# TinyMPC/TinyMPC

Measured on AMD Instinct MI355X. Metric: QP solves/sec (+ ADMM iters/sec), 64k-batch quadrotor hover, higher is better.
Workload: dtype f64; 1 GPU; quadrotor_hovering (nx=12, nu=4, N=10), 65536 identical instances per GPU, closed-loop MPC steps from a cold start (BASELINE configs[1]); batch_per_gpu=65536, total_batch=65536, parallelism=batch-sharded x1, mpc_steps_per_launch=8, stats_exchange=none (one rank), launcher=plain process

## Files before the change

tinympc_amd/csrc/admm_kernel.hip.h:

```cpp
#pragma once
#include <hip/hip_runtime.h>
#include <stdint.h>

namespace tinympc_amd {

enum : int {
    VEC_CB = 0,
    VEC_CF = 1,
    VEC_QR = 2,
    VEC_SMASK = 3,
    VEC_NIM = 4,
    VEC_SOCFLAG = 5,
    VEC_CONE_BASE = 6,
    VEC_CONE_MU = 7,
    VEC_RHO = 8,
    VEC_LINFLAG = 9,
    VEC_TLINFLAG = 10,
    VEC_COUNT = 16,
};
struct LaneTab {
    int cols, lw;
    constexpr int MB() const { return 0; }
    constexpr int MF1() const { return cols * lw; }
    constexpr int MF2() const { return 2 * cols * lw; }
    constexpr int PT() const { return 3 * cols * lw; }
    constexpr int VEC() const { return 4 * cols * lw; }
    constexpr int BOUNDS() const { return VEC() + VEC_COUNT * lw; }
    constexpr int het_doubles() const { return BOUNDS(); }
    constexpr int lin_offset(int N) const { return BOUNDS() + 2 * N * lw; }
    constexpr int tlin_offset(int N, int kmax) const { return lin_offset(N) + 3 * kmax * lw; }
    constexpr int doubles(int N, int kmax) const { return tlin_offset(N, kmax) + 3 * N * kmax * lw; }
};
constexpr LaneTab ROW_TAB{16, 16};
enum : int {
    TAB_MB = ROW_TAB.MB(), TAB_MF1 = ROW_TAB.MF1(), TAB_MF2 = ROW_TAB.MF2(), TAB_PT = ROW_TAB.PT(), TAB_VEC = ROW_TAB.VEC(),
    TAB_BOUNDS = ROW_TAB.BOUNDS(),
};
enum : int { LIN_KMAX = 4, LIN_KMAX_BIG = 32 };
enum : int {
    ATAB_AT = 0,
    ATAB_DK = 256,
    ATAB_DP = 512,
    ATAB_DC1 = 768,
    ATAB_DC2 = 1024,
    ATAB_DOUBLES = 1280,
};
static inline int tab_lin_offset(int N) { return ROW_TAB.lin_offset(N); }
static inline int tab_tlin_offset(int N, int kmax = LIN_KMAX) { return ROW_TAB.tlin_offset(N, kmax); }
static inline int tab_doubles(int N, int kmax = LIN_KMAX) { return ROW_TAB.doubles(N, kmax); }

struct SolveArgs {
    const double* tab;
    const double* x0;
    const double* ref;
    double* prim;
    double* slack;
    double* dual;
    double* slack_prev;
    double* cslack;
    double* cdual;
    int4* status;
    double* resid;
    double* x0_next;
    double* dbg_qr;
    double* dbg_pd;
    uint2* accum;
    int* iter_log;
    double* u0_log;
    double rho, tol_pri, tol_dua;
    int batch, max_iter, check_termination;
    int steps;
    const double* traj;
    const int* traj_offsets;
    int traj_points, traj_step0;
    int reset_duals;
    const double* het_tabs;
    double *lslack, *ldual, *tlslack, *tldual;
    int n_lin, n_tlin;
    int cold, store_mask;
    const int* index;
    const int* count;
    int iter_base;
    int* next_index;
    int* next_count;
    double *arho, *aK, *aP, *aC1, *aC2;
    const double* atab;
    double arho_min, arho_max;
    int aclip;
    int ref_shared;
    int* work_counter;
    int reverse;
    const int* perm;
    int perm_count;
    double* vz_stream;
    int pf_mask, pf_shards, pf_static;
    union {
        unsigned* pf_counter;
        const double* inst_bounds;
        const double* inst_lin;
        const double* inst_cones;
    };
    unsigned pf_base[8];
};
static_assert(sizeof(SolveArgs) == 472 && __builtin_offsetof(SolveArgs, het_tabs) == 208 && __builtin_offsetof(SolveArgs, pf_mask) == 416 &&
              __builtin_offsetof(SolveArgs, pf_counter) == 432 && __builtin_offsetof(SolveArgs, pf_base) == 440, "SolveArgs: size and offsets are fixed");

#define DPP_FMA(acc, src, m, lane, bank) "v_fmac_f64_dpp %[" acc "], %[" src "], %[" m "] row_newbcast:" lane " row_mask:0xf bank_mask:" bank "\n\t"
#define DPP_REP1(S) S(0, 0)
#define DPP_REP2(S) DPP_REP1(S) S(1, 1)
#define DPP_REP3(S) DPP_REP2(S) S(2, 0)
#define DPP_REP4(S) DPP_REP3(S) S(3, 1)
#define DPP_REP5(S) DPP_REP4(S) S(4, 0)
#define DPP_REP6(S) DPP_REP5(S) S(5, 1)
#define DPP_REP7(S) DPP_REP6(S) S(6, 0)
#define DPP_REP8(S) DPP_REP7(S) S(7, 1)
#define DPP_REP9(S) DPP_REP8(S) S(8, 0)
#define DPP_REP10(S) DPP_REP9(S) S(9, 1)
#define DPP_REP11(S) DPP_REP10(S) S(10, 0)
#define DPP_REP12(S) DPP_REP11(S) S(11, 1)
#define DPP_REP13(S) DPP_REP12(S) S(12, 0)
#define DPP_REP14(S) DPP_REP13(S) S(13, 1)
#define DPP_REP15(S) DPP_REP14(S) S(14, 0)
#define DPP_REP16(S) DPP_REP15(S) S(15, 1)
#define DPP_REP_(K, S) DPP_REP##K(S)
#define DPP_REP(K, S) DPP_REP_(K, S)
#define DPP_ROW_M(k, p) , [m##k] "v"(m[k])
#define DPP_ROW_A(k, p) , [a##k] "v"(ma[k])
#define DPP_ROW_B(k, p) , [b##k] "v"(mb_[k])
#define RING2_COL(k, p) DPP_FMA("a" #p, "src", "m" #k, "%[c0]+" #k, "0xf")
#define RING1_COL(k, p) DPP_FMA("a0", "src", "m" #k, "%[c0]+" #k, "0xf")
#define RING_CASE(K)                                                                                                                     \
    if constexpr (NCOL == K)                                                                                                             \
        asm("s_nop 1\n\t" DPP_REP(K, RING2_COL) : [a0] "+&v"(a0), [a1] "+&v"(a1) : [src] "v"(src), [c0] "i"(COL0) DPP_REP(K, DPP_ROW_M));
#define RING1_CASE(K)                                                                                                                    \
    if constexpr (NCOL == K)                                                                                                             \
        asm("s_nop 1\n\t" DPP_REP(K, RING1_COL) : [a0] "+&v"(a0) : [src] "v"(src), [c0] "i"(COL0) DPP_REP(K, DPP_ROW_M));

template <int C>
__device__ __forceinline__ double row_bcast(double v) {
    int lo = __double2loint(v), hi = __double2hiint(v);
    lo = __builtin_amdgcn_update_dpp(0, lo, 0x150 + C, 0xf, 0xf, false);
    hi = __builtin_amdgcn_update_dpp(0, hi, 0x150 + C, 0xf, 0xf, false);
    return __hiloint2double(hi, lo);
}
template <int COL0, int NCOL, int K>
struct RingB {
    static __device__ __forceinline__ void run(double& a0, double& a1, double src, const double* m) {
        if constexpr (K < NCOL) {
            if constexpr ((K & 1) == 0) a0 = fma(row_bcast<COL0 + K>(src), m[K], a0);
            else a1 = fma(row_bcast<COL0 + K>(src), m[K], a1);
            RingB<COL0, NCOL, K + 1>::run(a0, a1, src, m);
        }
    }
};

template <int MODE, int COL0, int NCOL>
__device__ __forceinline__ void ring(double& a0, double& a1, double src, const double* m) {
    static_assert(NCOL >= 1 && NCOL <= 16 && COL0 + NCOL <= 16, "one DPP row");
    if constexpr (MODE == 0) {
        RING_CASE(1) RING_CASE(2) RING_CASE(3) RING_CASE(4) RING_CASE(5) RING_CASE(6) RING_CASE(7) RING_CASE(8)
        RING_CASE(9) RING_CASE(10) RING_CASE(11) RING_CASE(12) RING_CASE(13) RING_CASE(14) RING_CASE(15) RING_CASE(16)
    } else {
        RingB<COL0, NCOL, 0>::run(a0, a1, src, m);
    }
}
template <int COL0, int NCOL>
__device__ __forceinline__ void ring1(double& a0, double src, const double* m) {
    static_assert(NCOL >= 1 && NCOL <= 16 && COL0 + NCOL <= 16, "one DPP row");
    RING1_CASE(1) RING1_CASE(2) RING1_CASE(3) RING1_CASE(4) RING1_CASE(5) RING1_CASE(6) RING1_CASE(7) RING1_CASE(8)
    RING1_CASE(9) RING1_CASE(10) RING1_CASE(11) RING1_CASE(12) RING1_CASE(13) RING1_CASE(14) RING1_CASE(15) RING1_CASE(16)
}
template <int MODE, int NA, int NB>
__device__ __forceinline__ double ring_sum2(double init, double srcA, const double* mA, double srcB, const double* mB) {
    if constexpr (MODE == 2) {
        double a0 = init;
        ring1<0, NA>(a0, srcA, mA);
        ring1<NA, NB>(a0, srcB, mB);
        return a0;
    } else {
        double a0 = init, a1 = 0.0;
        ring<MODE, 0, NA>(a0, a1, srcA, mA);
        ring<MODE, NA, NB>(a0, a1, srcB, mB);
        return a0 + a1;
    }
}
template <int MODE, int COL0, int NCOL>
__device__ __forceinline__ double ring_sum(double init, double src, const double* m) {
    if constexpr (MODE == 2) {
        double a0 = init;
        ring1<COL0, NCOL>(a0, src, m);
        return a0;
    } else {
        double a0 = init, a1 = 0.0;
        ring<MODE, COL0, NCOL>(a0, a1, src, m);
        return a0 + a1;
    }
}
template <int MODE, int COL0, int NCOL>
__device__ __forceinline__ double ring_short(double init, double src, const double* m) {
    if constexpr (MODE == 1) return ring_sum<1, COL0, NCOL>(init, src, m);
    else { double a0 = init; ring1<COL0, NCOL>(a0, src, m); return a0; }
}


#define RINGH_LO(k, p) DPP_FMA("a0", "src", "m" #k, "%[c0]+" #k, "0x3")
#define RINGH_HI(k, p) DPP_FMA("a0", "src", "m" #k, "8+%[c0]+" #k, "0xc")
#define RINGH_CASE(K)                                                                                                                    \
    if constexpr (NCOL == K)                                                                                                             \
        asm("s_nop 1\n\t" DPP_REP(K, RINGH_LO) "s_nop 0\n\t" DPP_REP(K, RINGH_HI) : [a0] "+&v"(a0) : [src] "v"(src), [c0] "i"(COL0) DPP_REP(K, DPP_ROW_M));
template <int COL0, int NCOL>
__device__ __forceinline__ void ring1_half(double& a0, double src, const double* m) {
    static_assert(NCOL >= 1 && COL0 + NCOL <= 8, "one half row");
    RINGH_CASE(1) RINGH_CASE(2) RINGH_CASE(3) RINGH_CASE(4) RINGH_CASE(5) RINGH_CASE(6) RINGH_CASE(7) RINGH_CASE(8)
}


#if defined(TINYMPC_FUSED_NX) && defined(TINYMPC_FUSED_NU)
#define TINYMPC_FUSED 1
constexpr bool fused_shape(int na, int nb) { return na == TINYMPC_FUSED_NX && nb == TINYMPC_FUSED_NU; }
#define FUSED_ROW_OPERANDS [c0] "i"(TINYMPC_FUSED_NX) DPP_REP(TINYMPC_FUSED_NX, DPP_ROW_A) DPP_REP(TINYMPC_FUSED_NU, DPP_ROW_B)
#else
constexpr bool fused_shape(int, int) { return false; }
#endif
#define BWD_COL_A(k, p) DPP_FMA("acc", "sa", "a" #k, #k, "0xf")
#define BWD_COL_B(k, p) DPP_FMA("acc", "sb", "b" #k, "%[c0]+" #k, "0xf")
#define FWD_COL_A(k, p) DPP_FMA("t", "xi", "a" #k, #k, "0xf")
#define FWD_COL_B(k, p) DPP_FMA("xn", "t", "b" #k, "%[c0]+" #k, "0xf")
#define FWD_COL_B_INPLACE(k, p) DPP_FMA("t", "t", "b" #k, "%[c0]+" #k, "%[bm]")
template <int NA, int NB>
__device__ __forceinline__ void fused_backward_step(double& qlo, double& acc, double vn, double g, double qx, double rho, double smask, double cb,
                                                    double sa, double sb, const double* ma, const double* mb_) {
#ifdef TINYMPC_FUSED
    if constexpr (fused_shape(NA, NB)) {
        double tmp;
        asm("v_add_f64 %[tmp], %[vn], -%[g]\n\t"
            "v_fma_f64 %[qlo], -%[rho], %[tmp], %[qx]\n\t"
            "v_fma_f64 %[acc], %[qlo], %[smask], %[cb]\n\t"
            DPP_REP(TINYMPC_FUSED_NX, BWD_COL_A) DPP_REP(TINYMPC_FUSED_NU, BWD_COL_B)
            : [qlo] "=&v"(qlo), [acc] "=&v"(acc), [tmp] "=&v"(tmp)
            : [vn] "v"(vn), [g] "v"(g), [qx] "v"(qx), [rho] "v"(rho), [smask] "v"(smask), [cb] "v"(cb), [sa] "v"(sa), [sb] "v"(sb), FUSED_ROW_OPERANDS);
    }
#endif
}
template <int NA, int NB>
__device__ __forceinline__ void fused_backward_step_soc(double& qlo, double& acc, double vn, double g, double qx, double w, double rho,
                                                        double smask, double cb, double sa, double sb, const double* ma, const double* mb_) {
#ifdef TINYMPC_FUSED
    if constexpr (fused_shape(NA, NB)) {
        double tmp;
        asm("v_add_f64 %[tmp], %[vn], -%[g]\n\t"
            "v_fma_f64 %[qlo], -%[rho], %[tmp], %[qx]\n\t"
            "v_fma_f64 %[qlo], -%[rho], %[w], %[qlo]\n\t"
            "v_fma_f64 %[acc], %[qlo], %[smask], %[cb]\n\t"
            DPP_REP(TINYMPC_FUSED_NX, BWD_COL_A) DPP_REP(TINYMPC_FUSED_NU, BWD_COL_B)
            : [qlo] "=&v"(qlo), [acc] "=&v"(acc), [tmp] "=&v"(tmp)
            : [vn] "v"(vn), [g] "v"(g), [qx] "v"(qx), [rho] "v"(rho), [smask] "v"(smask), [cb] "v"(cb), [sa] "v"(sa), [sb] "v"(sb),
              [w] "v"(w), FUSED_ROW_OPERANDS);
    }
#endif
}
template <int NA, int NB, bool INPLACE = false>
__device__ __forceinline__ void fused_forward_step(double& tt, double& vn, double& t, double& xn, double xi, double g, double lo, double hi,
                                                   const double* ma, const double* mb_) {
#ifdef TINYMPC_FUSED
    if constexpr (fused_shape(NA, NB) && !(INPLACE && TINYMPC_FUSED_NX % 4 == 0)) {
        double vm;
        asm("v_add_f64 %[tt], %[xi], %[g]\n\t"
            "v_max_f64 %[vm], %[lo], %[tt]\n\t"
            DPP_REP(TINYMPC_FUSED_NX, FWD_COL_A)
            "v_min_f64 %[vn], %[hi], %[vm]\n\t"
            "v_mov_b64 %[xn], %[t]\n\t"
            DPP_REP(TINYMPC_FUSED_NU, FWD_COL_B)
            : [tt] "=&v"(tt), [vm] "=&v"(vm), [vn] "=&v"(vn), [xn] "=&v"(xn), [t] "+&v"(t)
            : [xi] "v"(xi), [g] "v"(g), [lo] "v"(lo), [hi] "v"(hi), FUSED_ROW_OPERANDS);
    }
    if constexpr (fused_shape(NA, NB) && INPLACE && TINYMPC_FUSED_NX % 4 == 0) {
        asm("v_add_f64 %[tt], %[xi], %[g]\n\t"
            DPP_REP(TINYMPC_FUSED_NX, FWD_COL_A)
            "v_max_f64 %[vn], %[lo], %[tt]\n\t"
            "v_min_f64 %[vn], %[hi], %[vn]\n\t"
            DPP_REP(TINYMPC_FUSED_NU, FWD_COL_B_INPLACE)
            : [tt] "=&v"(tt), [vn] "=&v"(vn), [t] "+&v"(t)
            : [xi] "v"(xi), [g] "v"(g), [lo] "v"(lo), [hi] "v"(hi), [bm] "i"((1 << (TINYMPC_FUSED_NX / 4)) - 1), FUSED_ROW_OPERANDS);
        xn = t;
    }
#endif
}
#if defined(TINYMPC_FUSED) && TINYMPC_FUSED_NX + TINYMPC_FUSED_NU <= 8
#define TINYMPC_FUSED_HALF 1
#endif
#define HBWD_COL_A_LO(k, p) DPP_FMA("acc", "sa", "a" #k, #k, "0x3")
#define HBWD_COL_A_HI(k, p) DPP_FMA("acc", "sa", "a" #k, "8+" #k, "0xc")
#define HBWD_COL_B_LO(k, p) DPP_FMA("acc", "sb", "b" #k, "%[c0]+" #k, "0x3")
#define HBWD_COL_B_HI(k, p) DPP_FMA("acc", "sb", "b" #k, "8+%[c0]+" #k, "0xc")
#define HFWD_COL_A_LO(k, p) DPP_FMA("t", "xi", "a" #k, #k, "0x3")
#define HFWD_COL_A_HI(k, p) DPP_FMA("t", "xi", "a" #k, "8+" #k, "0xc")
#define HFWD_COL_B_LO(k, p) DPP_FMA("xn", "t", "b" #k, "%[c0]+" #k, "0x3")
#define HFWD_COL_B_HI(k, p) DPP_FMA("xn", "t", "b" #k, "8+%[c0]+" #k, "0xc")
template <int NA, int NB>
__device__ __forceinline__ void fused_backward_step_half(double& qlo, double& acc, double& dnp, double& tmpn, double tmp, double vnn, double gn, double qx,
                                                         double rho, double smask, double cb, double nim, double cf, double sa, double sb,
                                                         const double* ma, const double* mb_) {
#ifdef TINYMPC_FUSED_HALF
    if constexpr (fused_shape(NA, NB)) {
        asm("v_fma_f64 %[qlo], -%[rho], %[tmp], %[qx]\n\t"
            "v_fma_f64 %[acc], %[qlo], %[smask], %[cb]\n\t"
            "v_fma_f64 %[dnp], %[sa], %[nim], %[cf]\n\t"
            DPP_REP(TINYMPC_FUSED_NX, HBWD_COL_A_LO) DPP_REP(TINYMPC_FUSED_NU, HBWD_COL_B_LO)
            "v_add_f64 %[tmpn], %[vnn], -%[gn]\n\t"
            DPP_REP(TINYMPC_FUSED_NX, HBWD_COL_A_HI) DPP_REP(TINYMPC_FUSED_NU, HBWD_COL_B_HI)
            : [qlo] "=&v"(qlo), [acc] "=&v"(acc), [dnp] "=&v"(dnp), [tmpn] "=&v"(tmpn)
            : [tmp] "v"(tmp), [vnn] "v"(vnn), [gn] "v"(gn), [qx] "v"(qx), [rho] "v"(rho), [smask] "v"(smask), [cb] "v"(cb),
              [nim] "v"(nim), [cf] "v"(cf), [sa] "v"(sa), [sb] "v"(sb), FUSED_ROW_OPERANDS);
    }
#endif
}
template <int NA, int NB>
__device__ __forceinline__ void fused_forward_step_half(double& tt, double& vn, double& t, double& xn, double& gnew, double xi, double g,
                                                        double lo, double hi, const double* ma, const double* mb_) {
#ifdef TINYMPC_FUSED_HALF
    if constexpr (fused_shape(NA, NB)) {
        double vm;
        asm("v_add_f64 %[tt], %[xi], %[g]\n\t"
            "v_max_f64 %[vm], %[lo], %[tt]\n\t"
            DPP_REP(TINYMPC_FUSED_NX, HFWD_COL_A_LO)
            "v_min_f64 %[vn], %[hi], %[vm]\n\t"
            DPP_REP(TINYMPC_FUSED_NX, HFWD_COL_A_HI)
            "v_mov_b64 %[xn], %[t]\n\t"
            "v_add_f64 %[gnew], %[tt], -%[vn]\n\t"
            DPP_REP(TINYMPC_FUSED_NU, HFWD_COL_B_LO)
            "s_nop 0\n\t"
            DPP_REP(TINYMPC_FUSED_NU, HFWD_COL_B_HI)
            : [tt] "=&v"(tt), [vm] "=&v"(vm), [vn] "=&v"(vn), [xn] "=&v"(xn), [t] "+&v"(t), [gnew] "=&v"(gnew)
            : [xi] "v"(xi), [g] "v"(g), [lo] "v"(lo), [hi] "v"(hi), FUSED_ROW_OPERANDS);
    }
#endif
}

__device__ __forceinline__ double vmax64(double a, double b) {
    double r;
    asm("v_max_f64 %0, %1, %2" : "=v"(r) : "v"(a), "v"(b));
    return r;
}
__device__ __forceinline__ double vmin64(double a, double b) {
    double r;
    asm("v_min_f64 %0, %1, %2" : "=v"(r) : "v"(a), "v"(b));
    return r;
}
__device__ __forceinline__ double pinned_sub64(double a, double b) {
    double r = a - b;
    asm volatile("" : "+v"(r));
    return r;
}
__device__ __forceinline__ double vclamp64(double lo, double hi, double t) {
    double r;
    asm("v_max_f64 %0, %1, %2\n\tv_min_f64 %0, %3, %0" : "=&v"(r) : "v"(lo), "v"(t), "v"(hi));
    return r;
}

__device__ __forceinline__ double vmax_abs64(double a, double b) {
    double r;
    asm("v_max_f64 %0, %1, |%2|" : "=v"(r) : "v"(a), "v"(b));
    return r;
}
template <bool OPAQUE>
__device__ __forceinline__ double resid_max(double a, double b) {
    if constexpr (OPAQUE) return vmax_abs64(a, b);
    else return fmax(a, fabs(b));
}

#ifndef TINYMPC_PRIM_STORE
#define TINYMPC_PRIM_STORE 1
#endif
#ifndef TINYMPC_REF_LOAD
#define TINYMPC_REF_LOAD 1
#endif
#ifndef TINYMPC_FULL_LINE_STORES
#define TINYMPC_FULL_LINE_STORES 2
#endif
__device__ __forceinline__ double load_ref(const double* p) {
#if TINYMPC_REF_LOAD == 1
    return __builtin_nontemporal_load(p);
#else
    return *p;
#endif
}
__device__ __forceinline__ void store_primal(double* p, double v) {
#if TINYMPC_PRIM_STORE == 1
    __builtin_nontemporal_store(v, p);
#elif TINYMPC_PRIM_STORE == 2
    asm volatile("global_store_dwordx2 %0, %1, off sc1" : : "v"(p), "v"(v) : "memory");
#elif TINYMPC_PRIM_STORE == 3
    asm volatile("global_store_dwordx2 %0, %1, off sc0 sc1" : : "v"(p), "v"(v) : "memory");
#elif TINYMPC_PRIM_STORE == 4
    asm volatile("global_store_dwordx2 %0, %1, off sc0 sc1 nt" : : "v"(p), "v"(v) : "memory");
#else
    *p = v;
#endif
}

__device__ __forceinline__ double grp_max16(double v) {
#pragma unroll
    for (int off = 8; off >= 1; off >>= 1) v = fmax(v, __shfl_xor(v, off, 16));
    return v;
}
template <int W>
__device__ __forceinline__ double grp_maxw(double v) {
#pragma unroll
    for (int off = W / 2; off >= 1; off >>= 1) v = fmax(v, __shfl_xor(v, off, W));
    return v;
}

__device__ __forceinline__ bool soc_all_inside(double s0, double s1, double s2, float mu) {
#pragma clang fp contract(off)
    const double u0 = s2 * (double)mu;
    const double q0 = s0 * s0, q1 = s1 * s1;
    const double q = q0 + q1;
    const bool sure_inside = (u0 > 1e-30) & (u0 < 1e300) & (q <= (u0 * u0) * (1.0 - 0x1p-20)) & (q < 1e70);
    return __builtin_amdgcn_ballot_w64(!sure_inside) == 0ull;
}
__device__ __forceinline__ void soc_project3(double s0, double s1, double s2, float mu, float rmu, bool rmu_exact, double& r0, double& r1, double& r2) {
#pragma clang fp contract(off)
    const double u0 = s2 * (double)mu;
    const double q0 = s0 * s0, q1 = s1 * s1;
    const double q = q0 + q1;
    const float a = (float)sqrt(q);
    const double ad = (double)a;
    const bool below = ad <= -u0, inside = ad <= u0;
    const bool outside = !below && !inside && (ad >= fabs(u0));
    const bool zero = below || !inside;
    r0 = zero ? 0.0 : s0; r1 = zero ? 0.0 : s1; r2 = zero ? 0.0 : s2;
    if (__builtin_amdgcn_ballot_w64(outside) != 0ull) {
        const double scale = 0.5 * (1.0 + u0 / ad);
        const double last = (double)(rmu_exact ? a * rmu : a / mu);
        r0 = outside ? scale * s0 : r0;
        r1 = outside ? scale * s1 : r1;
        r2 = outside ? scale * last : r2;
    }
}
__device__ __forceinline__ int soc_items_of(unsigned heads, int nx, int n) {
    int c = 0;
    for (unsigned m = heads; m; m &= m - 1) c += (__builtin_ctz(m) < nx) ? n : n - 1;
    return c;
}
constexpr int soc_item_passes(int nx, int nu, int n) { return ((nx / 3) * n + (nu / 3) * (n - 1) + 15) / 16; }

constexpr int ADAPT_LOG = 32;
__device__ __forceinline__ double taylor_step(double a, double d, double b) {
#pragma clang fp contract(off)
    const double t = d * b;
    return a + t;
}

constexpr int solve_kernel_waves_per_simd(int nz, int n, bool soc, bool lin = false, bool adapt = false) {
    if (lin) return 1;
    if (adapt) return n <= 10 ? 2 : 1;
    return (n <= 10 || 2 * ((soc ? 8 : 6) * n + 2 * nz + 8) + 40 <= 256) ? 2 : 1;
}

#ifndef TINYMPC_LIN_WAVES
#define TINYMPC_LIN_WAVES 0
#endif
constexpr long solve_kernel_lin_lds(int nx, int nu, int n, bool soc, int lin, int kmax, bool ub, bool pl = false) {
    const int nz = nx + nu, csl = (nz + 1) | 1, cs = (nz + 1) | 1, tabs = pl ? 4 : 1;
    return 8L * (nx * 16 + (ub ? 2 : 2 * n * 16) + ((lin & 1) ? tabs * 3 * kmax * 16 + 2 * 4 * n * csl : 0) +
                 ((lin & 2) ? tabs * 3 * n * kmax * 16 + 2 * 4 * n * csl : 0) + (soc ? (4 * n + 1) * 3 * cs : 0));
}
constexpr bool solve_kernel_lin_planes(int nx, int nu, int n, bool soc, int lin, int kmax, bool ub, bool pl = false) {
    return lin != 0 && solve_kernel_lin_lds(nx, nu, n, soc, lin, kmax, ub, pl) <= 64 * 1024 - 512;
}
constexpr int solve_kernel_lin_waves(int nx, int nu, int n, bool soc, int lin, int kmax, bool ub, bool pl = false) {
    if (!solve_kernel_lin_planes(nx, nu, n, soc, lin, kmax, ub, pl)) return 1;
    if (TINYMPC_LIN_WAVES > 0) return TINYMPC_LIN_WAVES;
    return (solve_kernel_waves_per_simd(nx + nu, n, soc) == 2 && 8 * solve_kernel_lin_lds(nx, nu, n, soc, lin, kmax, ub, pl) <= 158 * 1024) ? 2 : 1;
}
template <int NF, int KMAX_, int LW_, int LPI_>
__device__ __forceinline__ void project_halfspace_columns(const int t, const int inst, const int n, const int csl, const int R0, const int S0,
                                                          double* pv, double* pg, const double* tab, const int tab_stride, const int nk) {
#pragma clang fp contract(off)
    for (int c = S0 + t; c < n; c += LPI_) {
        const int at = (inst * n + c) * csl + R0;
        const double* tk = tab + c * tab_stride;
        double z[NF], t0[NF];
#pragma unroll
        for (int r = 0; r < NF; ++r) { z[r] = pv[at + r]; t0[r] = z[r]; }
        for (int k = 0; k < nk; ++k) {
            double cv = 0.0;
#pragma unroll
            for (int r = 0; r < NF; ++r) { const double pr = tk[k * LW_ + R0 + r] * z[r]; cv = cv + pr; }
            const double bk = tk[KMAX_ * LW_ + k * LW_ + R0];
            if (cv > bk) {
                const double dist = (cv - bk) / tk[2 * KMAX_ * LW_ + k * LW_ + R0];
#pragma unroll
                for (int r = 0; r < NF; ++r) { const double pr = dist * tk[k * LW_ + R0 + r]; z[r] = z[r] - pr; }
            }
        }
#pragma unroll
        for (int r = 0; r < NF; ++r) { pv[at + r] = z[r]; pg[at + r] = t0[r] - z[r]; }
    }
}

template <int NX, int NU, int N, bool SOC, bool DBG, int MODE_PB, int LIN = 0, bool HET = false, int KMAX = LIN_KMAX, bool ADAPT = false, bool UB = false, bool HALF = false,
          bool PF = false>
__global__ __launch_bounds__(64)
__attribute__((amdgpu_waves_per_eu(LIN != 0 ? solve_kernel_lin_waves(NX, NU, N, SOC, LIN, KMAX, UB, (MODE_PB & 8) != 0) : solve_kernel_waves_per_simd(NX + NU, N, SOC, false, ADAPT),
                                   LIN != 0 ? solve_kernel_lin_waves(NX, NU, N, SOC, LIN, KMAX, UB, (MODE_PB & 8) != 0) : solve_kernel_waves_per_simd(NX + NU, N, SOC, false, ADAPT))))
void admm_solve_kernel(const SolveArgs P) {
    constexpr int MODE = MODE_PB & 3;
    constexpr bool PB = (MODE_PB & 4) != 0;
    constexpr bool PL = (MODE_PB & 8) != 0;
    constexpr bool PC = (MODE_PB & 16) != 0;
    static_assert(MODE <= 2 && MODE_PB < 32, "MODE 0 | 1 | 2, + 4: per-instance box, + 8: per-instance half-spaces, + 16: per-instance cone coefficients");
    static_assert(!PC || SOC, "per-instance cone coefficients: a cone variant (SOC)");
    static_assert(!PC || (!PL && !ADAPT), "per-instance cone coefficients: not with per-instance half-spaces (coverage kernel) or adaptive rho (refused)");
    static_assert(!PL || LIN != 0, "per-instance half-spaces: a half-space variant (LIN != 0)");
    static_assert(!PL || !HALF, "per-instance half-spaces: not the half-row form");
    static_assert(!PL || !PF, "per-instance half-spaces: not the prefetch form");
    static_assert(!PL || !ADAPT, "per-instance half-spaces: not with adaptive rho (refused, as on shared half-spaces)");
    static_assert(!PL || !PB, "per-instance half-spaces: not with a per-instance box (that combination runs on the coverage kernel)");
    static_assert(!PL || solve_kernel_lin_planes(NX, NU, N, SOC, LIN, KMAX, UB, true),
                  "per-instance half-spaces: the slack planes and the four rows' tables must fit the wave's static LDS");
    constexpr bool LS = (LIN & 1) != 0, LT = (LIN & 2) != 0;
    constexpr int NZ = NX + NU;
    static_assert(NZ <= 16, "one instance per 16-lane DPP row");
    constexpr bool FUSED = MODE == 2 && LIN == 0 && fused_shape(NX, NU);
    static_assert(!HALF || (NZ <= 8 && FUSED && !SOC && !DBG && !HET && !ADAPT), "half rows: nx+nu <= 8, the plain box kernel on its fused step blocks");
    static_assert(!PF || (MODE == 2 && !SOC && !DBG && LIN == 0 && !HET && !ADAPT), "prefetch form: the plain box kernel");
    static_assert(!PB || (!HALF && !PF), "per-instance box: full rows, not the prefetch form");
    static_assert(!PB || UB || 4L * solve_kernel_waves_per_simd(NX + NU, N, SOC, false, ADAPT) * (128 * NX + 1024 * N) <= 160 * 1024,
                  "per-instance box: the rows' bound blocks must leave the shape its waves per SIMD");
    static_assert(!PB || (!SOC && LIN == 0 && !ADAPT), "per-instance box: the box variants (cones, half-spaces and adaptive rho run on the coverage kernel / are refused)");
    constexpr int RL = HALF ? 8 : 16;
    constexpr int IPW = 64 / RL;
    constexpr int RECD = N * NZ;
    constexpr int PF_PIECES = (IPW * RECD * 8 + 1023) / 1024;
    constexpr int PF_ARR = PF_PIECES * 128;
    constexpr unsigned long long RMASK = HALF ? 0xFFull : 0xFFFFull;
    const int lane = threadIdx.x & 63;
    const int j = lane & (RL - 1);
    const int grp = lane / RL;
    const bool is_state = j < NX;
    const bool is_input = (j >= NX) && (j < NZ);

    __shared__ double sPt[NX * 16];
    __shared__ double sLo[UB ? 1 : (PB ? IPW : 1) * N * 16];
    __shared__ double sHi[UB ? 1 : (PB ? IPW : 1) * N * 16];
    __shared__ double sLin[LS ? (PL ? IPW : 1) * 3 * KMAX * 16 : 1];
    __shared__ double sTLin[LT ? (PL ? IPW : 1) * 3 * N * KMAX * 16 : 1];
#ifndef TINYMPC_SOC_PD
#define TINYMPC_SOC_PD 2
#endif
    constexpr int SPD = TINYMPC_SOC_PD, SPR = SPD + 1;
    constexpr int CS = SOC ? ((NZ + 1) | 1) : 1;
    constexpr int SLOT_D = 3 * CS;
    constexpr int PL_GC = CS, PL_VC = 2 * CS;
    __shared__ double sC[SOC ? (4 * N + 1) * SLOT_D : 1];
    __shared__ double sP[ADAPT ? 4 * NX * NX : 1];
    constexpr int AKC = NX > NU ? NX : NU;
    constexpr bool HA = HET && ADAPT;
    __shared__ double sTab[(ADAPT && !HET) ? 3 * 16 * AKC : 1];
    __shared__ double sDl[ADAPT ? 4 * ADAPT_LOG : 1];
    if constexpr (ADAPT && !HET)
        for (int e = lane; e < 3 * 16 * AKC; e += 64) {
            const int t = e / (16 * AKC), r = e % (16 * AKC);
            sTab[e] = P.atab[t * 256 + (r % AKC) * 16 + r / AKC];
        }
    if constexpr (LS && !PL) for (int e = lane; e < 3 * KMAX * 16; e += 64) sLin[e] = P.tab[TAB_BOUNDS + 2 * N * 16 + e];
    if constexpr (LT && !PL) for (int e = lane; e < 3 * N * KMAX * 16; e += 64) sTLin[e] = P.tab[TAB_BOUNDS + 2 * N * 16 + 3 * KMAX * 16 + e];
    for (int e = lane; e < NX * 16; e += 64) sPt[e] = P.tab[TAB_PT + e];
    for (int e = lane; e < N * 16; e += 64) {
        if constexpr (!UB && !PB) {
            sLo[e] = P.tab[TAB_BOUNDS + e];
            sHi[e] = P.tab[TAB_BOUNDS + N * 16 + e];
        }
    }
    double mb[NZ], mf1[NX], mf2[NU];
#pragma unroll
    for (int k = 0; k < NZ; ++k) mb[k] = P.tab[TAB_MB + k * 16 + j];
#pragma unroll
    for (int k = 0; k < NX; ++k) mf1[k] = P.tab[TAB_MF1 + k * 16 + j];
#pragma unroll
    for (int k = 0; k < NU; ++k) mf2[k] = P.tab[TAB_MF2 + (NX + k) * 16 + j];
    double cb = P.tab[TAB_VEC + VEC_CB * 16 + j];
    double cf = P.tab[TAB_VEC + VEC_CF * 16 + j];
    double qr = P.tab[TAB_VEC + VEC_QR * 16 + j];
    const double smask = PB ? (is_state ? 1.0 : 0.0) : P.tab[TAB_VEC + VEC_SMASK * 16 + j];
    const double nim = PB ? (is_input ? -1.0 : 0.0) : P.tab[TAB_VEC + VEC_NIM * 16 + j];
    bool soc_lane = false, proj_lane = false;
    int cone_base = -1, cone_c = 0;
    double socmask = 0.0;
    if constexpr (SOC) {
        socmask = P.tab[TAB_VEC + VEC_SOCFLAG * 16 + j];
        soc_lane = socmask != 0.0;
        cone_base = (int)P.tab[TAB_VEC + VEC_CONE_BASE * 16 + j];
        cone_c = (cone_base >= 0) ? (j - cone_base) : 0;
        proj_lane = soc_lane && cone_base >= 0;
    }
    constexpr int SOC_PASSES = SOC ? (soc_item_passes(NX, NU, N) > 0 ? soc_item_passes(NX, NU, N) : 1) : 1;
    int item_at[SOC_PASSES];
    float item_mu[SOC_PASSES], item_rmu[SOC_PASSES];
    bool mu_pow2 = !PC;
    int soc_passes = 0;
    if constexpr (SOC) {
        if (lane < 3) {
            sC[4 * N * SLOT_D + lane] = lane == 2 ? 1.0 : 0.0;
            sC[4 * N * SLOT_D + PL_GC + lane] = 0.0;
            sC[4 * N * SLOT_D + PL_VC + lane] = lane == 2 ? 1.0 : 0.0;
        }
        const unsigned heads = (unsigned)(__builtin_amdgcn_ballot_w64(proj_lane && cone_c == 0) & 0xFFFFull);
#pragma unroll
        for (int p = 0; p < SOC_PASSES; ++p) {
            int t = p * 16 + j;
            item_at[p] = 4 * N * SLOT_D; item_mu[p] = 1.0f;
            if (heads && p * 16 < soc_items_of(heads, NX, N)) soc_passes = p + 1;
            for (unsigned m = heads; m; m &= m - 1) {
                const int hb = __builtin_ctz(m);
                const int cnt = hb < NX ? N : N - 1;
                if (t >= 0 && t < cnt) {
                    item_at[p] = (grp * N + t + (hb < NX ? 0 : 1)) * SLOT_D + hb;
                    if constexpr (!PC) item_mu[p] = (float)P.tab[TAB_VEC + VEC_CONE_MU * 16 + hb];
                    t = -1;
                } else if (t >= 0) t -= cnt;
            }
            item_rmu[p] = 1.0f / item_mu[p];
            if constexpr (!PC) {
                const unsigned mb_ = __float_as_uint(item_mu[p]);
                const bool p2 = (mb_ & 0x807FFFFFu) == 0u && (mb_ >> 23) >= 127u - 60u && (mb_ >> 23) <= 127u + 60u;
                if (__builtin_amdgcn_ballot_w64(!p2) != 0ull) mu_pow2 = false;
            }
        }
    }
    bool lin_lane = false, tlin_lane = false;
    if constexpr (LS) lin_lane = P.tab[TAB_VEC + VEC_LINFLAG * 16 + j] != 0.0;
    if constexpr (LT) tlin_lane = P.tab[TAB_VEC + VEC_TLINFLAG * 16 + j] != 0.0;
    constexpr bool LPL = solve_kernel_lin_planes(NX, NU, N, SOC, LIN, KMAX, UB, PL);
    constexpr bool LSP = LS && LPL, LTP = LT && LPL, LSR = LS && !LPL, LTR = LT && !LPL;
    constexpr int CSL = LPL ? ((NZ + 1) | 1) : 1;
    __shared__ double sLV[LSP ? 4 * N * CSL : 1], sLG[LSP ? 4 * N * CSL : 1];
    __shared__ double sTV[LTP ? 4 * N * CSL : 1], sTG[LTP ? 4 * N * CSL : 1];
    double ones[(LSR || LTR) ? 16 : 1];
#pragma unroll
    for (int k = 0; k < ((LSR || LTR) ? 16 : 1); ++k) ones[k] = 1.0;
    bool lin_x_on = false, lin_u_on = false, tlin_x_on = false, tlin_u_on = false;
    if constexpr (LS) { lin_x_on = P.tab[TAB_VEC + VEC_LINFLAG * 16] != 0.0; lin_u_on = P.tab[TAB_VEC + VEC_LINFLAG * 16 + NX] != 0.0; }
    if constexpr (LT) { tlin_x_on = P.tab[TAB_VEC + VEC_TLINFLAG * 16] != 0.0; tlin_u_on = P.tab[TAB_VEC + VEC_TLINFLAG * 16 + NX] != 0.0; }
    double rho = P.rho;
    __builtin_amdgcn_fence(__ATOMIC_RELEASE, "wavefront");
    __builtin_amdgcn_wave_barrier();

    const double lo_u = PB ? 0.0 : P.tab[TAB_BOUNDS + (N > 1 ? 16 : 0) + j], hi_u = PB ? 0.0 : P.tab[TAB_BOUNDS + N * 16 + (N > 1 ? 16 : 0) + j];
    const double lo_u0 = PB ? 0.0 : P.tab[TAB_BOUNDS + j], hi_u0 = PB ? 0.0 : P.tab[TAB_BOUNDS + N * 16 + j];
    const int sbox = PB ? grp * (N * 16) : 0;
    const double* const rLin = sLin + (PL ? grp * (3 * KMAX * 16) : 0);
    const double* const rTLin = sTLin + (PL ? grp * (3 * N * KMAX * 16) : 0);
    const int ninst = PF ? P.batch : (P.index ? *P.count : (P.perm ? P.perm_count : P.batch));
    const int ntiles = (ninst + IPW - 1) / IPW;
    const bool resumed = !PF && P.index != nullptr;
    const bool has_traj = !PF && P.traj != nullptr;
    extern __shared__ __attribute__((aligned(16))) double sPF[];
    typedef const __attribute__((address_space(1))) void* pf_gptr;
    typedef __attribute__((address_space(3))) void* pf_lptr;
    constexpr int PF_S0 = 128, PF_S1 = PF_S0 + PF_ARR, PF_S2 = PF_S1 + PF_ARR, PF_S3 = PF_S2 + PF_ARR;
    auto pf_issue = [&](const int t) {
        const int tl = P.reverse ? ntiles - 1 - t : t;
        __builtin_amdgcn_global_load_lds((pf_gptr)(P.x0 + ((size_t)tl * (IPW * NX) + (size_t)lane * 2)), (pf_lptr)sPF, 16, 0, 0);
        const size_t t0 = (size_t)tl * (IPW * RECD) + (size_t)lane * 2;
        auto arr = [&](const double* p, const int at) {
#pragma unroll
            for (int q = 0; q < PF_PIECES; ++q) __builtin_amdgcn_global_load_lds((pf_gptr)(p + t0 + q * 128), (pf_lptr)(sPF + at + q * 128), 16, 0, 0);
        };
        if (!P.cold) { arr(P.slack, PF_S0); arr(P.dual, PF_S1); arr(P.slack_prev, PF_S2); }
        if (P.pf_mask & 8) arr(P.ref, P.cold ? PF_S0 : PF_S3);
    };
    unsigned pf_ticket = 0u;
    const int pf_shard = PF ? (int)(blockIdx.x % (unsigned)(P.pf_shards > 0 ? P.pf_shards : 1)) : 0;
    typedef __attribute__((address_space(1))) unsigned* pf_ctr_t;
    unsigned long long pf_ctr_bits = PF ? (unsigned long long)(P.pf_counter + 16 * pf_shard) : 0ull;
    if constexpr (PF) asm volatile("" : "+v"(pf_ctr_bits));
    const pf_ctr_t pf_ctr = (pf_ctr_t)pf_ctr_bits;
    auto pf_draw = [&]() { return lane == 0 ? __hip_atomic_fetch_add(pf_ctr, 1u, __ATOMIC_RELAXED, __HIP_MEMORY_SCOPE_AGENT) : 0u; };
    const unsigned pf_base = PF ? P.pf_base[pf_shard] : 0u;
    int pf_next = 0, pf_i = 0;
    bool pf_first = true;
    double* const sQX = sPF + PF_S3;
    if constexpr (PF) {
        if ((int)blockIdx.x < ntiles) {
            pf_issue((int)blockIdx.x);
            if (P.pf_static <= 1) pf_ticket = pf_draw();
        }
        if (P.ref_shared) {
            double rl = 0.0, qxs[N];
#pragma unroll
            for (int s = 0; s < N; ++s) {
                const bool valid = is_state || (is_input && s >= 1);
                const double r = valid ? P.ref[j - (is_input ? NZ : 0) + s * NZ] : 0.0;
                qxs[s] = -(r * qr);
                if (s == N - 1) rl = r;
            }
            double pt[NX];
#pragma unroll
            for (int k = 0; k < NX; ++k) pt[k] = sPt[k * 16 + j];
            double xp = 0.0;
            if constexpr (HALF) ring1_half<0, NX>(xp, rl, pt);
            else xp = ring_sum<MODE, 0, NX>(0.0, rl, pt);
            qxs[N - 1] = is_state ? -xp : qxs[N - 1];
            if (grp == 0) {
#pragma unroll
                for (int s = 0; s < N; ++s) sQX[s * 16 + j] = qxs[s];
            }
            __builtin_amdgcn_fence(__ATOMIC_RELEASE, "wavefront");
            __builtin_amdgcn_wave_barrier();
        }
    }
    for (int tile = blockIdx.x; tile < ntiles;
         tile = PF ? pf_next : (P.work_counter ? __builtin_amdgcn_readfirstlane(lane == 0 ? atomicAdd(P.work_counter, 1) : 0) + (int)gridDim.x : tile + (int)gridDim.x)) {
        const int slot = (P.reverse ? ntiles - 1 - tile : tile) * IPW + grp;
        double pfVN[PF ? N : 1], pfG[PF ? N : 1], pfVP[PF ? N : 1], pfQXs[PF ? N : 1], pf_x0 = 0.0, pf_rl = 0.0;
        if constexpr (PF) {
            if (pf_first) asm volatile("s_waitcnt vmcnt(0)" ::: "memory");
            else if ((P.store_mask & 6) == 6) asm volatile("s_waitcnt vmcnt(%0)" :: "n"(2 * N <= 63 ? 2 * N : 63) : "memory");
            else asm volatile("s_waitcnt vmcnt(0)" ::: "memory");
            pf_first = false;
            if (pf_i + 1 < P.pf_static) pf_next = tile + (int)gridDim.x;
            else {
                unsigned pf_t;
                asm volatile("v_readfirstlane_b32 %0, %1" : "=s"(pf_t) : "v"(pf_ticket));
                pf_next = (int)(pf_t - pf_base) * P.pf_shards + pf_shard + (P.pf_static > 1 ? P.pf_static : 1) * (int)gridDim.x;
            }
            const int m = P.pf_mask;
            const int lrow = grp * RECD + (j < NZ ? j - (is_input ? NZ : 0) : 0);
            const bool warm_t = !P.cold;
            pf_x0 = sPF[grp * NX + (is_state ? j : 0)];
#pragma unroll
            for (int s = 0; s < N; ++s) { pfVN[s] = 0.0; pfG[s] = 0.0; pfVP[s] = 0.0; }
            if (warm_t) {
#pragma unroll
                for (int s = 0; s < N; ++s) { pfVN[s] = sPF[PF_S0 + lrow + s * NZ]; pfG[s] = sPF[PF_S1 + lrow + s * NZ]; }
            }
            auto own_ref = [&](const int at) {
#pragma unroll
                for (int s = 0; s < N; ++s) {
                    const bool valid = is_state || (is_input && s >= 1);
                    const double r = valid ? sPF[at + lrow + s * NZ] : 0.0;
                    pfQXs[s] = -(r * qr);
                    if (s == N - 1) pf_rl = r;
                }
            };
            if (m & 8) { if (warm_t) own_ref(PF_S3); else own_ref(PF_S0); }
            else {
#pragma unroll
                for (int s = 0; s < N; ++s) pfQXs[s] = sQX[s * 16 + j];
            }
            if (warm_t) {
#pragma unroll
                for (int s = 0; s < N; ++s) pfVP[s] = sPF[PF_S2 + lrow + s * NZ];
            }
            asm volatile("s_waitcnt lgkmcnt(0)" ::: "memory");
            if (pf_next < ntiles) {
                if (pf_i + 2 >= P.pf_static) {
                    asm volatile("" ::: "memory");
                    pf_ticket = pf_draw();
                }
                pf_issue(pf_next);
            }
            ++pf_i;
        }
        (void)pfVN; (void)pfG; (void)pfVP; (void)pf_rl; (void)pf_x0; (void)pfQXs; (void)pf_first; (void)pf_ticket; (void)sQX; (void)pf_ctr; (void)pf_base; (void)pf_draw; (void)pf_i;
        if (slot < ninst) {
            const int b = PF ? slot : (resumed ? P.index[slot] : (P.perm ? P.perm[slot] : slot));
            const double* het = nullptr;
            if constexpr (HET) {
                het = P.het_tabs + (size_t)b * TAB_BOUNDS;
#pragma unroll
                for (int k = 0; k < NZ; ++k) mb[k] = het[TAB_MB + k * 16 + j];
#pragma unroll
                for (int k = 0; k < NX; ++k) mf1[k] = het[TAB_MF1 + k * 16 + j];
#pragma unroll
                for (int k = 0; k < NU; ++k) mf2[k] = het[TAB_MF2 + (NX + k) * 16 + j];
                cb = het[TAB_VEC + VEC_CB * 16 + j];
                cf = het[TAB_VEC + VEC_CF * 16 + j];
                qr = het[TAB_VEC + VEC_QR * 16 + j];
                rho = het[TAB_VEC + VEC_RHO * 16 + j];
            }
            double rlo_u = lo_u, rhi_u = hi_u, rlo_u0 = lo_u0, rhi_u0 = hi_u0;
            if constexpr (PB) {
                size_t ib_at = (size_t)b * (2 * N * 16) + j;
                asm volatile("" : "+v"(ib_at));
                const double* ib = P.inst_bounds + ib_at;
                if constexpr (UB) {
                    rlo_u0 = ib[0]; rhi_u0 = ib[N * 16];
                    rlo_u = ib[N > 1 ? 16 : 0]; rhi_u = ib[N * 16 + (N > 1 ? 16 : 0)];
                } else {
#pragma unroll
                    for (int s = 0; s < N; ++s) { sLo[sbox + s * 16 + j] = ib[s * 16]; sHi[sbox + s * 16 + j] = ib[N * 16 + s * 16]; }
                    __builtin_amdgcn_fence(__ATOMIC_RELEASE, "wavefront");
                    __builtin_amdgcn_wave_barrier();
                }
            }
            if constexpr (PL) {
                constexpr int LBLK = 3 * KMAX * 16;
                size_t il_at = (size_t)b * ((LS ? LBLK : 0) + (LT ? N * LBLK : 0)) + j;
                asm volatile("" : "+v"(il_at));
                const double* il = P.inst_lin + il_at;
                if constexpr (LS) {
#pragma unroll
                    for (int e = 0; e < 3 * KMAX; ++e) sLin[grp * LBLK + e * 16 + j] = il[e * 16];
                }
                if constexpr (LT) {
                    const double* ilt = il + (LS ? LBLK : 0);
                    for (int e = 0; e < 3 * KMAX * N; ++e) sTLin[grp * (N * LBLK) + e * 16 + j] = ilt[e * 16];
                }
                __builtin_amdgcn_fence(__ATOMIC_RELEASE, "wavefront");
                __builtin_amdgcn_wave_barrier();
            }
            if constexpr (PC) {
                size_t ic_at = (size_t)b * 16;
                asm volatile("" : "+v"(ic_at));
                const double* ic = P.inst_cones + ic_at;
#pragma unroll
                for (int p = 0; p < SOC_PASSES; ++p) {
                    int at = item_at[p];
                    asm volatile("" : "+v"(at));
                    const bool has = at != 4 * N * SLOT_D;
                    const float own = (float)ic[has ? at % SLOT_D : 0];
                    item_mu[p] = has ? own : 1.0f;
                }
            }
            if constexpr (ADAPT) {
                rho = P.arho[b];
                const double* aK = P.aK + (size_t)b * (NU * NX);
                if (is_state) {
#pragma unroll
                    for (int k = 0; k < NU; ++k) mb[NX + k] = -aK[k + NU * j];
#pragma unroll
                    for (int k = 0; k < NX; ++k) sP[grp * NX * NX + k + NX * j] = P.aP[(size_t)b * (NX * NX) + k + NX * j];
                } else if (is_input) {
#pragma unroll
                    for (int k = 0; k < NX; ++k) mf1[k] = -aK[(j - NX) + NU * k];
                }
                __builtin_amdgcn_fence(__ATOMIC_RELEASE, "wavefront");
                __builtin_amdgcn_wave_barrier();
            }
            const double* atab_i = nullptr;
            if constexpr (HET && ADAPT) atab_i = P.atab + (size_t)b * ATAB_DOUBLES;
            (void)atab_i;
            const size_t lbase = (size_t)b * (N * NZ) + j - (is_input ? NZ : 0);
            double X[N], G[N], VN[N], VP[N], QX[N], Dn[N - 1];
            const int cw = grp * N * SLOT_D + (j < NZ ? j : NZ);
            const double x0v_in = is_state ? (PF ? pf_x0 : P.x0[(size_t)b * NX + j]) : 0.0;
            const int cl = grp * N * CSL + (j < NZ ? j : NZ);
            double VL[LSR ? N : 1], GL[LSR ? N : 1], VT[LTR ? N : 1], GT[LTR ? N : 1];
            double Qd[DBG ? N : 1], Pd[DBG ? N : 1], Dd[DBG ? N : 1];
            double ref_last = 0.0, qx_last_plain = 0.0;
#pragma unroll
            for (int s = 0; s < N; ++s) {
                const bool valid = is_state || (is_input && s >= 1);
                const size_t off = lbase + s * NZ;
                const bool warm = valid && !P.cold;
                if constexpr (PF) {
                    VN[s] = warm ? pfVN[s] : 0.0;
                    G[s] = warm ? pfG[s] : 0.0;
                    VP[s] = warm ? pfVP[s] : 0.0;
                    QX[s] = pfQXs[s];
                    X[s] = 0.0;
                    if (s == N - 1) ref_last = pf_rl;
                    continue;
                }
                const double r = valid ? (P.ref_shared ? P.ref[off - (size_t)b * (N * NZ)] : load_ref(P.ref + off)) : 0.0;
                VN[s] = warm ? P.slack[off] : 0.0;
                G[s] = warm ? P.dual[off] : 0.0;
                VP[s] = warm ? P.slack_prev[off] : 0.0;
                QX[s] = -(r * qr);
                X[s] = 0.0;
                if (s == N - 1) ref_last = r;
                if constexpr (SOC) {
                    double vc0 = (warm && soc_lane) ? (resumed ? P.cslack : P.prim)[off] : 0.0;
                    const double gc0 = (warm && soc_lane) ? P.cdual[off] : 0.0;
                    if (s == 0 && is_state && soc_lane && !resumed) vc0 = x0v_in;
                    sC[cw + s * SLOT_D] = vc0 - gc0;
                    sC[cw + s * SLOT_D + PL_GC] = gc0;
                    sC[cw + s * SLOT_D + PL_VC] = vc0;
                }
                if constexpr (LS) {
                    const double vl0 = (warm && lin_lane) ? (resumed ? P.lslack : P.prim)[off] : 0.0;
                    const double gl0 = (warm && lin_lane) ? P.ldual[off] : 0.0;
                    if constexpr (LSP) { sLV[cl + s * CSL] = vl0; sLG[cl + s * CSL] = gl0; } else { VL[s] = vl0; GL[s] = gl0; }
                }
                if constexpr (LT) {
                    const double vt0 = (warm && tlin_lane) ? (resumed ? P.tlslack : P.prim)[off] : 0.0;
                    const double gt0 = (warm && tlin_lane) ? P.tldual[off] : 0.0;
                    if constexpr (LTP) { sTV[cl + s * CSL] = vt0; sTG[cl + s * CSL] = gt0; } else { VT[s] = vt0; GT[s] = gt0; }
                }
                if constexpr (DBG) { Qd[s] = 0.0; Pd[s] = 0.0; Dd[s] = 0.0; }
            }
            double x0v = x0v_in;
            auto terminal_term = [&]() {
                double pt[NX];
#pragma unroll
                for (int k = 0; k < NX; ++k)
                    pt[k] = ADAPT ? sP[grp * NX * NX + k + NX * (is_state ? j : 0)] : (HET ? het[TAB_PT + k * 16 + j] : sPt[k * 16 + j]);
                double xp = 0.0;
                if constexpr (HALF) ring1_half<0, NX>(xp, ref_last, pt);
                else xp = ring_sum<MODE, 0, NX>(0.0, ref_last, pt);
                qx_last_plain = QX[N - 1];
                QX[N - 1] = is_state ? -xp : QX[N - 1];
            };
            int ndl = 0;
            auto flush_c = [&](int n) {
                __builtin_amdgcn_fence(__ATOMIC_RELEASE, "wavefront");
                __builtin_amdgcn_wave_barrier();
                if (P.aC2 && is_state) {
                    double* c2 = P.aC2 + (size_t)b * (NX * NX) + NX * j;
                    double v[NX], d[NX];
#pragma unroll
                    for (int k = 0; k < NX; ++k) { v[k] = c2[k]; d[k] = P.atab[(HA ? (size_t)b * ATAB_DOUBLES : (size_t)0) + ATAB_DC2 + k * 16 + j]; }
                    for (int i = 0; i < n; ++i) {
                        const double dl = sDl[grp * ADAPT_LOG + i];
#pragma unroll
                        for (int k = 0; k < NX; ++k) v[k] = taylor_step(v[k], dl, d[k]);
                    }
#pragma unroll
                    for (int k = 0; k < NX; ++k) c2[k] = v[k];
                }
                if (P.aC1 && j < NU) {
                    double* c1 = P.aC1 + (size_t)b * (NU * NU) + NU * j;
                    double v[NU], d[NU];
#pragma unroll
                    for (int k = 0; k < NU; ++k) { v[k] = c1[k]; d[k] = P.atab[(HA ? (size_t)b * ATAB_DOUBLES : (size_t)0) + ATAB_DC1 + k * 16 + j]; }
                    for (int i = 0; i < n; ++i) {
                        const double dl = sDl[grp * ADAPT_LOG + i];
#pragma unroll
                        for (int k = 0; k < NU; ++k) v[k] = taylor_step(v[k], dl, d[k]);
                    }
#pragma unroll
                    for (int k = 0; k < NU; ++k) c1[k] = v[k];
                }
            };
            if (!has_traj && !(PF && P.ref_shared)) terminal_term();
            const int traj_k0 = has_traj ? (P.traj_step0 + (P.traj_offsets ? P.traj_offsets[b] : 0)) : 0;

            int iter = 0, solved = 0, checked = 0;
            unsigned acc_iter = 0, acc_solved = 0;
            bool vp_touched = false;
            double rp = 0.0, rd = 0.0;
            const int nsteps = PF ? 1 : (P.steps > 1 ? P.steps : 1);
            const int iter_first = resumed ? P.iter_base : 0;
            for (int step = 0; step < nsteps; ++step) {
                X[0] = x0v;
                if (has_traj) {
                    if (is_state) {
#pragma unroll
                        for (int s = 0; s < N; ++s) {
                            int kk = traj_k0 + step + s;
                            kk = kk < P.traj_points ? kk : P.traj_points - 1;
                            const double r = P.traj[(size_t)kk * NX + j];
                            QX[s] = -(r * qr);
                            if (s == N - 1) ref_last = r;
                        }
                    }
                    terminal_term();
                }
                if (P.reset_duals) {
#pragma unroll
                    for (int s = 0; s < N; ++s) G[s] = 0.0;
                }
                if constexpr (SOC) {
                    if (step > 0) {
#pragma unroll
                        for (int s = 0; s < N; ++s) {
                            const double vc0 = soc_lane ? X[s] : 0.0;
                            sC[cw + s * SLOT_D] = vc0 - sC[cw + s * SLOT_D + PL_GC];
                            sC[cw + s * SLOT_D + PL_VC] = vc0;
                        }
                    }
                }
                if constexpr (LS) {
                    if (step > 0) {
#pragma unroll
                        for (int s = 0; s < N; ++s) { if constexpr (LSP) sLV[cl + s * CSL] = lin_lane ? X[s] : 0.0; else VL[s] = lin_lane ? X[s] : 0.0; }
                    } else if (is_state && lin_lane && !resumed) { if constexpr (LSP) sLV[cl] = x0v; else VL[0] = x0v; }
                }
                if constexpr (LT) {
                    if (step > 0) {
#pragma unroll
                        for (int s = 0; s < N; ++s) { if constexpr (LTP) sTV[cl + s * CSL] = tlin_lane ? X[s] : 0.0; else VT[s] = tlin_lane ? X[s] : 0.0; }
                    } else if (is_state && tlin_lane && !resumed) { if constexpr (LTP) sTV[cl] = x0v; else VT[0] = x0v; }
                }
                if constexpr (LPL) __builtin_amdgcn_fence(__ATOMIC_RELEASE, "wavefront");
                const int iter0 = iter_first;
                iter = iter0; solved = 0;
                if (resumed && P.check_termination > 0) checked = 1;
                int countdown = P.check_termination;
                double wr[SOC ? SPR : 1];
                bool gcz[SOC_PASSES];
#pragma unroll
                for (int p = 0; p < SOC_PASSES; ++p) gcz[p] = false;
                if constexpr (SOC) {
#pragma unroll
                    for (int d = 1; d <= SPR && d <= N; ++d) wr[(N - d) % SPR] = sC[cw + (N - d) * SLOT_D];
                }
                for (int it = iter0; it < P.max_iter; ++it) {
                    double lvr[LSP ? SPR : 1], lgr[LSP ? SPR : 1], tvr[LTP ? SPR : 1], tgr[LTP ? SPR : 1];
                    if constexpr (LPL) {
#pragma unroll
                        for (int d = 1; d <= SPR && d <= N; ++d) {
                            if constexpr (LSP) { lvr[(N - d) % SPR] = sLV[cl + (N - d) * CSL]; lgr[(N - d) % SPR] = sLG[cl + (N - d) * CSL]; }
                            if constexpr (LTP) { tvr[(N - d) % SPR] = sTV[cl + (N - d) * CSL]; tgr[(N - d) % SPR] = sTG[cl + (N - d) * CSL]; }
                        }
                    }
                    auto lin_w = [&](const int s_) { if constexpr (LSP) return lvr[s_ % SPR] - lgr[s_ % SPR]; else return VL[LSR ? s_ : 0] - GL[LSR ? s_ : 0]; };
                    auto tlin_w = [&](const int s_) { if constexpr (LTP) return tvr[s_ % SPR] - tgr[s_ % SPR]; else return VT[LTR ? s_ : 0] - GT[LTR ? s_ : 0]; };
                    double qhi;
                    {
                        double t = fma(-rho, VN[N - 1] - G[N - 1], QX[N - 1]);
                        if constexpr (SOC) t = fma(-rho, wr[(N - 1) % SPR], t);
                        if constexpr (LS) t = fma(-rho, lin_w(N - 1), t);
                        if constexpr (LT) t = fma(-rho, tlin_w(N - 1), t);
                        qhi = t;
                        if constexpr (DBG) {
                            double ql = fma(-rho, VN[N - 1] - G[N - 1], qx_last_plain);
                            if constexpr (SOC) ql = fma(-rho, wr[(N - 1) % SPR], ql);
                            if constexpr (LS) ql = fma(-rho, lin_w(N - 1), ql);
                            if constexpr (LT) ql = fma(-rho, tlin_w(N - 1), ql);
                            Qd[N - 1] = is_state ? ql : t;
                            Pd[N - 1] = t;
                        }
                    }
                    double pcur = qhi;
                    if constexpr (HALF) {
                        double tmpv = VN[N - 2] - G[N - 2];
#pragma unroll
                        for (int i = N - 2; i >= 0; --i) {
                            double qlo, res, dnp, tmpn;
                            constexpr int dummy = 0;
                            const int in = i > 0 ? i - 1 : dummy;
                            fused_backward_step_half<NX, NU>(qlo, res, dnp, tmpn, tmpv, VN[in], G[in], QX[i], rho, smask, cb, nim, cf, pcur, qhi, mb, mb + NX);
                            if (i + 1 <= N - 2) Dn[i + 1] = dnp;
                            tmpv = tmpn;
                            pcur = res;
                            qhi = qlo;
                        }
                        Dn[0] = fma(pcur, nim, cf);
                    }
#pragma unroll
                    for (int i = N - 2; i >= 0 && !HALF; --i) {
                        if constexpr (SOC) {
                            if (i >= SPD) wr[(i - SPD) % SPR] = sC[cw + (i - SPD) * SLOT_D];
                        }
                        if constexpr (LSP) { if (i >= SPD) { lvr[(i - SPD) % SPR] = sLV[cl + (i - SPD) * CSL]; lgr[(i - SPD) % SPR] = sLG[cl + (i - SPD) * CSL]; } }
                        if constexpr (LTP) { if (i >= SPD) { tvr[(i - SPD) % SPR] = sTV[cl + (i - SPD) * CSL]; tgr[(i - SPD) % SPR] = sTG[cl + (i - SPD) * CSL]; } }
                        if constexpr (SOC || LPL) __builtin_amdgcn_sched_barrier(0);
                        if constexpr (FUSED) {
                            double qlo, res;
                            if constexpr (SOC) fused_backward_step_soc<NX, NU>(qlo, res, VN[i], G[i], QX[i], wr[i % SPR], rho, smask, cb, pcur, qhi, mb, mb + NX);
                            else fused_backward_step<NX, NU>(qlo, res, VN[i], G[i], QX[i], rho, smask, cb, pcur, qhi, mb, mb + NX);
                            pcur = res;
                            Dn[i] = fma(res, nim, cf);
                            if constexpr (DBG) { Qd[i] = qlo; Pd[i] = res; Dd[i + 1] = res; }
                            qhi = qlo;
                            continue;
                        }
                        double qlo = fma(-rho, VN[i] - G[i], QX[i]);
                        if constexpr (SOC) qlo = fma(-rho, wr[i % SPR], qlo);
                        if constexpr (LS) qlo = fma(-rho, lin_w(i), qlo);
                        if constexpr (LT) qlo = fma(-rho, tlin_w(i), qlo);
                        const double res = ring_sum2<MODE, NX, NU>(fma(qlo, smask, cb), pcur, mb, qhi, mb + NX);
                        pcur = res;
                        Dn[i] = fma(res, nim, cf);
                        if constexpr (DBG) { Qd[i] = qlo; Pd[i] = res; Dd[i + 1] = res; }
                        qhi = qlo;
                    }
                    constexpr bool LAZY_RES = N <= 12;
                    constexpr bool TIGHT = FUSED && !HALF && LAZY_RES && !SOC && NX % 4 == 0;
                    double pmax = 0.0, dmax = 0.0;
                    auto slot_update = [&](const int s, const double lo, const double hi, const double gcv, const double glv, const double gtv) {
                        const double xi = X[s];
                        const double t = xi + G[s];
                        const double vn = TIGHT ? vclamp64(lo, hi, t) : vmin64(hi, vmax64(lo, t));
                        if constexpr (!LAZY_RES) {
                            pmax = resid_max<true>(pmax, xi - vn);
                            dmax = resid_max<true>(dmax, VP[s] - vn);
                        }
                        G[s] = t - vn;
                        VN[s] = vn;
                        if constexpr (SOC) {
                            sC[cw + s * SLOT_D] = fma(xi, socmask, gcv);
                        }
                        if constexpr (LSP) sLV[cl + s * CSL] = (lin_lane && (is_state || s >= 1)) ? (xi + glv) : 0.0;
                        if constexpr (LTP) sTV[cl + s * CSL] = (tlin_lane && (is_state || s >= 1)) ? (xi + gtv) : 0.0;
                        if constexpr (LSR || LTR) {
                            auto halfspaces = [&](double z, const double* tabk, const int nk) {
                                for (int k = 0; k < nk; ++k) {
                                    const double a = tabk[k * 16 + j];
                                    const double bk = tabk[KMAX * 16 + k * 16 + j];
                                    const double nn = tabk[2 * KMAX * 16 + k * 16 + j];
                                    const double prod = a * z;
                                    double cs = 0.0, ci = 0.0;
                                    ring1<0, NX>(cs, prod, ones);
                                    ring1<NX, NU>(ci, prod, ones);
                                    const double cv = is_state ? cs : ci;
                                    if (cv > bk) {
#pragma clang fp contract(off)
                                        const double pr = ((cv - bk) / nn) * a;
                                        z = z - pr;
                                    }
                                }
                                return z;
                            };
                            if constexpr (LSR) {
                                const bool on = lin_lane && (is_state || s >= 1);
                                double vl = on ? (xi + GL[s]) : 0.0;
                                vl = halfspaces(vl, rLin, P.n_lin);
                                GL[s] = on ? ((GL[s] + xi) - vl) : 0.0;
                                VL[s] = on ? vl : 0.0;
                            }
                            if constexpr (LTR) {
                                const bool on = tlin_lane && (is_state || s >= 1);
                                double vt = on ? (xi + GT[s]) : 0.0;
                                vt = halfspaces(vt, rTLin + s * 3 * KMAX * 16, P.n_tlin);
                                GT[s] = on ? ((GT[s] + xi) - vt) : 0.0;
                                VT[s] = on ? vt : 0.0;
                            }
                        }
                    };
                    double lo_c = UB ? rlo_u0 : sLo[sbox + j], hi_c = UB ? rhi_u0 : sHi[sbox + j];
                    double gr[SOC ? SPR : 1];
                    if constexpr (SOC) {
#pragma unroll
                        for (int d = 0; d < SPD && d < N; ++d) gr[d % SPR] = sC[cw + d * SLOT_D + PL_GC];
                    } else gr[0] = 0.0;
                    double glr[LSP ? SPR : 1], gtr[LTP ? SPR : 1];
                    glr[0] = 0.0; gtr[0] = 0.0;
                    if constexpr (LPL) {
#pragma unroll
                        for (int d = 0; d < SPD && d < N; ++d) {
                            if constexpr (LSP) glr[d % SPR] = sLG[cl + d * CSL];
                            if constexpr (LTP) gtr[d % SPR] = sTG[cl + d * CSL];
                        }
                    }
                    double tt_d = 0.0, vn_d = 0.0;
#pragma unroll
                    for (int i = 0; i < N - 1; ++i) {
                        const double lo_n = UB ? rlo_u : sLo[sbox + (i + 1) * 16 + j], hi_n = UB ? rhi_u : sHi[sbox + (i + 1) * 16 + j];
                        if constexpr (SOC) { if (i + SPD < N) gr[(i + SPD) % SPR] = sC[cw + (i + SPD) * SLOT_D + PL_GC]; }
                        if constexpr (LSP) { if (i + SPD < N) glr[(i + SPD) % SPR] = sLG[cl + (i + SPD) * CSL]; }
                        if constexpr (LTP) { if (i + SPD < N) gtr[(i + SPD) % SPR] = sTG[cl + (i + SPD) * CSL]; }
                        __builtin_amdgcn_sched_barrier(0);
                        if constexpr (FUSED) {
                            double tt, vn, xn, t = Dn[i];
                            const double xi = X[i];
                            if constexpr (HALF) {
                                double gnew;
                                fused_forward_step_half<NX, NU>(tt, vn, t, xn, gnew, xi, G[i], lo_c, hi_c, mf1, mf2);
                                X[i + 1] = xn;
                                if constexpr (!LAZY_RES) {
                                    pmax = resid_max<true>(pmax, xi - vn);
                                    dmax = resid_max<true>(dmax, VP[i] - vn);
                                }
                                G[i] = gnew;
                                VN[i] = vn;
                                lo_c = lo_n; hi_c = hi_n;
                                continue;
                            }
                            fused_forward_step<NX, NU, TIGHT>(tt, vn, t, xn, xi, G[i], lo_c, hi_c, mf1, mf2);
                            X[i + 1] = xn;
                            if constexpr (!LAZY_RES) {
                                pmax = resid_max<true>(pmax, xi - vn);
                                dmax = resid_max<true>(dmax, VP[i] - vn);
                            }
                            if constexpr (TIGHT) {
                                __builtin_amdgcn_sched_barrier(0);
                                if (i > 0) G[i - 1] = pinned_sub64(tt_d, vn_d);
                                tt_d = tt; vn_d = vn;
                            } else G[i] = tt - vn;
                            VN[i] = vn;
                            if constexpr (SOC) sC[cw + i * SLOT_D] = fma(xi, socmask, gr[i % SPR]);
                            lo_c = lo_n; hi_c = hi_n;
                            continue;
                        }
                        const double t = ring_sum<MODE, 0, NX>(Dn[i], X[i], mf1);
                        X[i + 1] = ring_short<MODE, NX, NU>(t, t, mf2);
                        slot_update(i, lo_c, hi_c, gr[SOC ? i % SPR : 0], glr[LSP ? i % SPR : 0], gtr[LTP ? i % SPR : 0]);
                        lo_c = lo_n; hi_c = hi_n;
                    }
                    if constexpr (TIGHT && N >= 2) G[N - 2] = tt_d - vn_d;
                    (void)tt_d; (void)vn_d;
                    slot_update(N - 1, lo_c, hi_c, gr[SOC ? (N - 1) % SPR : 0], glr[LSP ? (N - 1) % SPR : 0], gtr[LTP ? (N - 1) % SPR : 0]);
                    if constexpr (LPL) {
                        __builtin_amdgcn_fence(__ATOMIC_RELEASE, "wavefront");
                        __builtin_amdgcn_wave_barrier();
                        if constexpr (LSP) {
                            if (lin_x_on) project_halfspace_columns<NX, KMAX, 16, 16>(j, grp, N, CSL, 0, 0, sLV, sLG, rLin, 0, P.n_lin);
                            if (lin_u_on) project_halfspace_columns<NU, KMAX, 16, 16>(j, grp, N, CSL, NX, 1, sLV, sLG, rLin, 0, P.n_lin);
                        }
                        if constexpr (LTP) {
                            if (tlin_x_on) project_halfspace_columns<NX, KMAX, 16, 16>(j, grp, N, CSL, 0, 0, sTV, sTG, rTLin, 3 * KMAX * 16, P.n_tlin);
                            if (tlin_u_on) project_halfspace_columns<NU, KMAX, 16, 16>(j, grp, N, CSL, NX, 1, sTV, sTG, rTLin, 3 * KMAX * 16, P.n_tlin);
                        }
                        __builtin_amdgcn_fence(__ATOMIC_RELEASE, "wavefront");
                        __builtin_amdgcn_wave_barrier();
                    }
                    bool conv = false;
                    auto termination = [&]() {
                        if (countdown > 0 && --countdown == 0) {
                            countdown = P.check_termination;
                            checked = 1;
                            constexpr int PS0 = N >= 2 ? 1 : 0, PS1 = N - 1;
                            auto lost = [&](const int s) {
                                return (int)(fabs(X[s] - VN[s]) >= P.tol_pri) | (int)(fabs(VP[s] - VN[s]) * rho >= P.tol_dua);
                            };
                            const bool maybe = ((int)!(rho > 0.0) | (int)!(lost(PS0) | lost(PS1))) != 0;
                            unsigned long long fold = __ballot(maybe);
                            fold &= fold >> 1; fold &= fold >> 2; fold &= fold >> 4;
                            if constexpr (!HALF) fold &= fold >> 8;
                            const bool any_row = (fold & (HALF ? 0x0101010101010101ull : 0x0001000100010001ull)) != 0ull;
                            const bool last_test = (P.max_iter - 1 - it) < P.check_termination;
                            if (last_test || any_row) {
                                if constexpr (LAZY_RES) {
#pragma unroll
                                    for (int s = 0; s < N; ++s) {
                                        pmax = resid_max<false>(pmax, X[s] - VN[s]);
                                        dmax = resid_max<false>(dmax, VP[s] - VN[s]);
                                    }
                                }
                                rp = pmax;
                                rd = dmax * rho;
                                const bool ok = (rp < P.tol_pri) && (rd < P.tol_dua);
                                const unsigned long long bal = __ballot(ok);
                                conv = ((bal >> (grp * RL)) & RMASK) == RMASK;
                            }
                        }
                    };
                    if constexpr (SOC) {
                        __builtin_amdgcn_fence(__ATOMIC_RELEASE, "wavefront");
                        __builtin_amdgcn_wave_barrier();
                        double n0 = sC[item_at[0]], n1 = sC[item_at[0] + 1], n2 = sC[item_at[0] + 2];
#pragma unroll
                        for (int d = 1; d <= SPR && d <= N; ++d) wr[(N - d) % SPR] = sC[cw + (N - d) * SLOT_D];
                        termination();
                        bool any_exact = false;
#pragma unroll
                        for (int p = 0; p < SOC_PASSES; ++p) {
                            if (p > 0 && p >= soc_passes) break;
                            const int at = item_at[p];
                            if (p > 0) { n0 = sC[at]; n1 = sC[at + 1]; n2 = sC[at + 2]; }
                            const double s0 = n0, s1 = n1, s2 = n2;
                            if (soc_all_inside(s0, s1, s2, item_mu[p])) {
                                sC[at + PL_VC] = s0; sC[at + PL_VC + 1] = s1; sC[at + PL_VC + 2] = s2;
                                if (!gcz[p]) {
                                    sC[at + PL_GC] = 0.0; sC[at + PL_GC + 1] = 0.0; sC[at + PL_GC + 2] = 0.0;
                                    gcz[p] = true;
                                }
                            } else {
                                double r0, r1, r2;
                                soc_project3(s0, s1, s2, item_mu[p], item_rmu[p], mu_pow2, r0, r1, r2);
                                const double g0 = s0 - r0, g1 = s1 - r1, g2 = s2 - r2;
                                sC[at + PL_VC] = r0; sC[at + PL_VC + 1] = r1; sC[at + PL_VC + 2] = r2;
                                sC[at + PL_GC] = g0; sC[at + PL_GC + 1] = g1; sC[at + PL_GC + 2] = g2;
                                sC[at] = r0 - g0; sC[at + 1] = r1 - g1; sC[at + 2] = r2 - g2;
                                gcz[p] = false;
                                any_exact = true;
                            }
                        }
                        if (it == iter0 && !proj_lane) {
#pragma unroll
                            for (int s = 0; s < N; ++s) sC[cw + s * SLOT_D + PL_GC] = 0.0;
                        }
                        __builtin_amdgcn_fence(__ATOMIC_RELEASE, "wavefront");
                        __builtin_amdgcn_wave_barrier();
                        if (any_exact) {
#pragma unroll
                            for (int d = 1; d <= SPR && d <= N; ++d) wr[(N - d) % SPR] = sC[cw + (N - d) * SLOT_D];
                        }
                    }
                    iter += 1;
                    if constexpr (ADAPT) {
                        if (it > 0 && it % 5 == 0) {
                            double at[NX];
#pragma unroll
                            for (int k = 0; k < NX; ++k) at[k] = HA ? atab_i[ATAB_AT + k * 16 + j] : sTab[j * AKC + k];
                            double pri_res = 0.0, ax_max = 0.0, z_max = 0.0, dual_res = 0.0, px_max = 0.0, aty_max = 0.0, q_max = 0.0;
                            double pxq_max = 0.0;
#pragma unroll
                            for (int i = 0; i < N - 1; ++i) {
                                const double axs = ring_sum<MODE, 0, NX>(0.0, X[i], mf1);
                                const double dyn = ring_short<MODE, NX, NU>(axs, is_input ? X[i + 1] : 0.0, mf2) - X[i + 1];
                                const double a = is_state ? dyn : X[i + 1];
                                const double zz = VN[i + 1];
                                const bool on = is_state || is_input;
                                pri_res = fmax(pri_res, on ? fabs(a - zz) : 0.0);
                                ax_max = fmax(ax_max, on ? fabs(a) : 0.0);
                                z_max = fmax(z_max, on ? fabs(zz) : 0.0);
                                const double init = is_state ? (i >= 1 ? -G[i] : 0.0) : G[i + 1];
                                const double aty = ring_sum<MODE, 0, NX>(init, G[i + 1], at);
                                const double xs = is_state ? X[i] : X[i + 1];
                                const double px = qr * xs;
                                dual_res = fmax(dual_res, on ? fabs((px + px) + aty) : 0.0);
                                pxq_max = fmax(pxq_max, on ? fabs(px) : 0.0);
                                aty_max = fmax(aty_max, on ? fabs(aty) : 0.0);
                            }
                            {
                                double prow[NX];
#pragma unroll
                                for (int k = 0; k < NX; ++k) prow[k] = sP[grp * NX * NX + (is_state ? j : 0) + NX * k];
                                const double pxl = ring_sum<MODE, 0, NX>(0.0, X[N - 1], prow);
                                const double ql = qr * X[N - 1];
                                const double atyl = -G[N - 1];
                                dual_res = fmax(dual_res, is_state ? fabs((pxl + ql) + atyl) : 0.0);
                                px_max = fmax(pxq_max, is_state ? fabs(pxl) : 0.0);
                                aty_max = fmax(aty_max, is_state ? fabs(atyl) : 0.0);
                                q_max = fmax(pxq_max, is_state ? fabs(ql) : 0.0);
                            }
                            pri_res = grp_max16(pri_res); ax_max = grp_max16(ax_max); z_max = grp_max16(z_max);
                            dual_res = grp_max16(dual_res); px_max = grp_max16(px_max); aty_max = grp_max16(aty_max); q_max = grp_max16(q_max);
                            const double pri_norm = fmax(ax_max, z_max);
                            const double dual_norm = fmax(fmax(px_max, aty_max), q_max);
                            const double eps = 1e-10;
                            const double normalized_pri = pri_res / (pri_norm + eps);
                            const double normalized_dual = dual_res / (dual_norm + eps);
                            const double ratio = normalized_pri / (normalized_dual + eps);
                            double new_rho = rho * sqrt(ratio);
                            if (P.aclip) new_rho = fmin(fmax(new_rho, P.arho_min), P.arho_max);
                            const double delta = new_rho - rho;
                            if (is_state) {
#pragma unroll
                                for (int k = 0; k < NU; ++k) mb[NX + k] = -taylor_step(-mb[NX + k], delta, (HA ? atab_i[ATAB_DK + k * 16 + j] : sTab[(16 + j) * AKC + k]));
#pragma unroll
                                for (int k = 0; k < NX; ++k) {
                                    const int e = grp * NX * NX + k + NX * j;
                                    sP[e] = taylor_step(sP[e], delta, (HA ? atab_i[ATAB_DP + k * 16 + j] : sTab[(32 + j) * AKC + k]));
                                }
                            } else if (is_input) {
#pragma unroll
                                for (int k = 0; k < NX; ++k) mf1[k] = -taylor_step(-mf1[k], delta, (HA ? atab_i[ATAB_DK + k * 16 + j] : sTab[(16 + j) * AKC + k]));
                            }
                            if (P.aC1 || P.aC2) {
                                if (j == 0) sDl[grp * ADAPT_LOG + ndl] = delta;
                                if (++ndl == ADAPT_LOG) { flush_c(ndl); ndl = 0; }
                            }
                            rho = new_rho;
                            __builtin_amdgcn_fence(__ATOMIC_RELEASE, "wavefront");
                            __builtin_amdgcn_wave_barrier();
                            QX[N - 1] = qx_last_plain;
                            terminal_term();
                        }
                    }
                    if constexpr (!SOC) termination();
                    if (conv) { solved = 1; break; }
#pragma unroll
                    for (int s = 0; s < N; ++s) VP[s] = VN[s];
                    vp_touched = true;
                }
                acc_iter += (unsigned)(iter - iter0);
                acc_solved += (unsigned)solved;
                if (P.iter_log && j == 0) P.iter_log[(size_t)step * P.batch + b] = solved ? iter : -iter;
                if (P.u0_log && is_input) P.u0_log[((size_t)step * P.batch + b) * NU + (j - NX)] = X[1];
                if (nsteps > 1) {
                    x0v = is_state ? X[1] : 0.0;
                }
            }

            constexpr bool FLS = TINYMPC_FULL_LINE_STORES != 0 && (PF || TINYMPC_FULL_LINE_STORES == 2) && !SOC && LIN == 0 && !DBG;
            if (FLS && (P.store_mask & 32) == 0) {
                if constexpr (FLS) {
                    const size_t seg = (size_t)b * (N * NZ) + j;
                    const bool in_row = j < NZ;
#pragma unroll
                    for (int s = 0; s < N; ++s) {
                        const size_t off = seg + s * NZ;
                        const double xs = is_input ? (s + 1 < N ? X[s + 1 < N ? s + 1 : s] : 0.0) : X[s];
                        const double vs = is_input ? (s + 1 < N ? VN[s + 1 < N ? s + 1 : s] : 0.0) : VN[s];
                        const double gs = is_input ? (s + 1 < N ? G[s + 1 < N ? s + 1 : s] : 0.0) : G[s];
                        const double ps = is_input ? (s + 1 < N ? VP[s + 1 < N ? s + 1 : s] : 0.0) : VP[s];
                        if (in_row) {
                            if (P.store_mask & 1) {
                                if (acc_iter > 0) { if constexpr (PF) P.prim[off] = xs; else store_primal(P.prim + off, xs); }
                                else if (s == 0 && is_state) P.prim[off] = xs;
                            }
                            if (P.store_mask & 2) P.slack[off] = vs;
                            if (P.store_mask & 4) P.dual[off] = gs;
                            if ((P.store_mask & 8) && vp_touched) P.slack_prev[off] = ps;
                        }
                    }
                }
            } else
#pragma unroll
            for (int s = 0; s < N; ++s) {
                const bool valid = is_state || (is_input && s >= 1);
                const size_t off = lbase + s * NZ;
                if (valid) {
                    if (((P.store_mask & 1) || ((P.store_mask & 32) && s <= 1)) && (acc_iter > 0 || (s == 0 && is_state))) {
                        if constexpr (SOC || LIN != 0) P.prim[off] = X[s];
                        else store_primal(P.prim + off, X[s]);
                    }
                    if (P.store_mask & 2) P.slack[off] = VN[s];
                    if (P.store_mask & 4) P.dual[off] = G[s];
                    if ((P.store_mask & 8) && vp_touched) P.slack_prev[off] = VP[s];
                    if constexpr (SOC) {
                        if (soc_lane && (P.store_mask & 16)) {
                            P.cslack[off] = sC[cw + s * SLOT_D + ((proj_lane || iter <= iter_first) ? PL_VC : 0)];
                            P.cdual[off] = sC[cw + s * SLOT_D + PL_GC];
                        }
                    }
                    if constexpr (LSP) { if (lin_lane && (P.store_mask & 16)) { P.lslack[off] = sLV[cl + s * CSL]; P.ldual[off] = sLG[cl + s * CSL]; } }
                    if constexpr (LTP) { if (tlin_lane && (P.store_mask & 16)) { P.tlslack[off] = sTV[cl + s * CSL]; P.tldual[off] = sTG[cl + s * CSL]; } }
                    if constexpr (LSR) { if (lin_lane && (P.store_mask & 16)) { P.lslack[off] = VL[s]; P.ldual[off] = GL[s]; } }
                    if constexpr (LTR) { if (tlin_lane && (P.store_mask & 16)) { P.tlslack[off] = VT[s]; P.tldual[off] = GT[s]; } }
                    if constexpr (DBG) {
                        if (P.dbg_qr && acc_iter > 0) {
                            P.dbg_qr[off] = Qd[s];
                            P.dbg_pd[off] = is_state ? Pd[s] : Dd[s];
                        }
                    }
                }
            }
            if constexpr (ADAPT) {
                if (ndl > 0) flush_c(ndl);
                if (j == 0) P.arho[b] = rho;
                if (is_state) {
#pragma unroll
                    for (int k = 0; k < NU; ++k) P.aK[(size_t)b * (NU * NX) + k + NU * j] = -mb[NX + k];
#pragma unroll
                    for (int k = 0; k < NX; ++k) P.aP[(size_t)b * (NX * NX) + k + NX * j] = sP[grp * NX * NX + k + NX * j];
                }
            }
            if (P.x0_next && acc_iter > 0 && is_state) P.x0_next[(size_t)b * NX + j] = X[1];
            const double ps = grp_maxw<RL>(is_state ? rp : 0.0), pi = grp_maxw<RL>(is_input ? rp : 0.0);
            const double ds = grp_maxw<RL>(is_state ? rd : 0.0), di = grp_maxw<RL>(is_input ? rd : 0.0);
            if (P.next_index) {
                const bool open = j == 0 && !solved;
                const unsigned long long m = __ballot(open);
                if (m) {
                    const int first = __ffsll((long long)m) - 1;
                    int at = 0;
                    if (lane == first) at = atomicAdd(P.next_count, __popcll(m));
                    at = __shfl(at, first);
                    if (open) P.next_index[at + __popcll(m & ((1ull << lane) - 1ull))] = b;
                }
            }
            if (j == 0) {
                P.status[b] = make_int4(iter, solved, solved ? 1 : 11, checked);
                double4 rr = make_double4(ps, pi, ds, di);
                *reinterpret_cast<double4*>(P.resid + (size_t)b * 4) = rr;
                if (P.accum) {
                    if constexpr (PF) {
                        __hip_atomic_fetch_add(&P.accum[b].x, acc_iter, __ATOMIC_RELAXED, __HIP_MEMORY_SCOPE_AGENT);
                        __hip_atomic_fetch_add(&P.accum[b].y, acc_solved, __ATOMIC_RELAXED, __HIP_MEMORY_SCOPE_AGENT);
                    } else {
                        uint2 ac = P.accum[b];
                        ac.x += acc_iter;
                        ac.y += acc_solved;
                        P.accum[b] = ac;
                    }
                }
            }
        }
    }
}

}
```

Measured before the change: 2.866 billion QP solves/s.

## Add wave-uniform inner ADMM loop with LDS-double-buffered previous slack and cheap probe termination

For the fused, non-SOC, box-only configuration, the ADMM iteration is wrapped in a tight do-while loop. The previous-slack vector VP moves from registers into a double-buffered LDS region, which drops the per-iteration register copy and frees VGPRs. Termination is split into a cheap probe that checks only two stages plus a ballot fold, and a full residual test that runs only when the probe fires. This is meant to cut per-iteration termination and copy overhead, at the cost of LDS traffic and more complex control flow that could drift from the exact termination semantics.

```diff
diff --git a/tinympc_amd/csrc/admm_kernel.hip.h b/tinympc_amd/csrc/admm_kernel.hip.h
--- a/tinympc_amd/csrc/admm_kernel.hip.h
+++ b/tinympc_amd/csrc/admm_kernel.hip.h
@@ -638,6 +638,8 @@
     constexpr int CSL = LPL ? ((NZ + 1) | 1) : 1;
     __shared__ double sLV[LSP ? 4 * N * CSL : 1], sLG[LSP ? 4 * N * CSL : 1];
     __shared__ double sTV[LTP ? 4 * N * CSL : 1], sTG[LTP ? 4 * N * CSL : 1];
+    constexpr bool UL = FUSED && !HALF && N <= 12 && !SOC && NX % 4 == 0 && !ADAPT && !DBG && !PF && UB;
+    __shared__ double sVP[UL ? 2 * N * 64 : 1];
     double ones[(LSR || LTR) ? 16 : 1];
 #pragma unroll
     for (int k = 0; k < ((LSR || LTR) ? 16 : 1); ++k) ones[k] = 1.0;
@@ -846,6 +848,10 @@
             (void)atab_i;
             const size_t lbase = (size_t)b * (N * NZ) + j - (is_input ? NZ : 0);
             double X[N], G[N], VN[N], VP[N], QX[N], Dn[N - 1];
+            int vcur = lane * 8;
+            constexpr int VSWAP = 64 * 8;
+            auto vp_cell = [&](const int at, const int s) { return reinterpret_cast<double*>(reinterpret_cast<char*>(sVP) + at) + s * 128; };
+            (void)vp_cell;
             const int cw = grp * N * SLOT_D + (j < NZ ? j : NZ);
             const double x0v_in = is_state ? (PF ? pf_x0 : P.x0[(size_t)b * NX + j]) : 0.0;
             const int cl = grp * N * CSL + (j < NZ ? j : NZ);
@@ -892,6 +898,10 @@
                     if constexpr (LTP) { sTV[cl + s * CSL] = vt0; sTG[cl + s * CSL] = gt0; } else { VT[s] = vt0; GT[s] = gt0; }
                 }
                 if constexpr (DBG) { Qd[s] = 0.0; Pd[s] = 0.0; Dd[s] = 0.0; }
+            }
+            if constexpr (UL) {
+#pragma unroll
+                for (int s = 0; s < N; ++s) *vp_cell(vcur, s) = VP[s];
             }
             double x0v = x0v_in;
             auto terminal_term = [&]() {
@@ -1000,356 +1010,419 @@
                     for (int d = 1; d <= SPR && d <= N; ++d) wr[(N - d) % SPR] = sC[cw + (N - d) * SLOT_D];
                 }
                 for (int it = iter0; it < P.max_iter; ++it) {
-                    double lvr[LSP ? SPR : 1], lgr[LSP ? SPR : 1], tvr[LTP ? SPR : 1], tgr[LTP ? SPR : 1];
-                    if constexpr (LPL) {
-#pragma unroll
-                        for (int d = 1; d <= SPR && d <= N; ++d) {
-                            if constexpr (LSP) { lvr[(N - d) % SPR] = sLV[cl + (N - d) * CSL]; lgr[(N - d) % SPR] = sLG[cl + (N - d) * CSL]; }
-                            if constexpr (LTP) { tvr[(N - d) % SPR] = sTV[cl + (N - d) * CSL]; tgr[(N - d) % SPR] = sTG[cl + (N - d) * CSL]; }
-                        }
-                    }
-                    auto lin_w = [&](const int s_) { if constexpr (LSP) return lvr[s_ % SPR] - lgr[s_ % SPR]; else return VL[LSR ? s_ : 0] - GL[LSR ? s_ : 0]; };
-                    auto tlin_w = [&](const int s_) { if constexpr (LTP) return tvr[s_ % SPR] - tgr[s_ % SPR]; else return VT[LTR ? s_ : 0] - GT[LTR ? s_ : 0]; };
-                    double qhi;
-                    {
-                        double t = fma(-rho, VN[N - 1] - G[N - 1], QX[N - 1]);
-                        if constexpr (SOC) t = fma(-rho, wr[(N - 1) % SPR], t);
-                        if constexpr (LS) t = fma(-rho, lin_w(N - 1), t);
-                        if constexpr (LT) t = fma(-rho, tlin_w(N - 1), t);
-                        qhi = t;
-                        if constexpr (DBG) {
-                            double ql = fma(-rho, VN[N - 1] - G[N - 1], qx_last_plain);
-                            if constexpr (SOC) ql = fma(-rho, wr[(N - 1) % SPR], ql);
-                            if constexpr (LS) ql = fma(-rho, lin_w(N - 1), ql);
-                            if constexpr (LT) ql = fma(-rho, tlin_w(N - 1), ql);
-                            Qd[N - 1] = is_state ? ql : t;
-                            Pd[N - 1] = t;
-                        }
-                    }
-                    double pcur = qhi;
-                    if constexpr (HALF) {
-                        double tmpv = VN[N - 2] - G[N - 2];
-#pragma unroll
-                        for (int i = N - 2; i >= 0; --i) {
-                            double qlo, res, dnp, tmpn;
-                            constexpr int dummy = 0;
-                            const int in = i > 0 ? i - 1 : dummy;
-                            fused_backward_step_half<NX, NU>(qlo, res, dnp, tmpn, tmpv, VN[in], G[in], QX[i], rho, smask, cb, nim, cf, pcur, qhi, mb, mb + NX);
-                            if (i + 1 <= N - 2) Dn[i + 1] = dnp;
-                            tmpv = tmpn;
-                            pcur = res;
-                            qhi = qlo;
-                        }
-                        Dn[0] = fma(pcur, nim, cf);
-                    }
-#pragma unroll
-                    for (int i = N - 2; i >= 0 && !HALF; --i) {
-                        if constexpr (SOC) {
-                            if (i >= SPD) wr[(i - SPD) % SPR] = sC[cw + (i - SPD) * SLOT_D];
-                        }
-                        if constexpr (LSP) { if (i >= SPD) { lvr[(i - SPD) % SPR] = sLV[cl + (i - SPD) * CSL]; lgr[(i - SPD) % SPR] = sLG[cl + (i - SPD) * CSL]; } }
-                        if constexpr (LTP) { if (i >= SPD) { tvr[(i - SPD) % SPR] = sTV[cl + (i - SPD) * CSL]; tgr[(i - SPD) % SPR] = sTG[cl + (i - SPD) * CSL]; } }
-                        if constexpr (SOC || LPL) __builtin_amdgcn_sched_barrier(0);
-                        if constexpr (FUSED) {
-                            double qlo, res;
-                            if constexpr (SOC) fused_backward_step_soc<NX, NU>(qlo, res, VN[i], G[i], QX[i], wr[i % SPR], rho, smask, cb, pcur, qhi, mb, mb + NX);
-                            else fused_backward_step<NX, NU>(qlo, res, VN[i], G[i], QX[i], rho, smask, cb, pcur, qhi, mb, mb + NX);
+                    constexpr bool LAZY_RES = N <= 12;
+                    constexpr bool TIGHT = FUSED && !HALF && LAZY_RES && !SOC && NX % 4 == 0;
+                    static_assert(!UL || TIGHT, "the wave-uniform loop is a form of the short box loop");
+                    constexpr int UPS0 = N >= 2 ? 1 : 0, UPS1 = N - 1;
+                    double vp0 = 0.0, vp1 = 0.0;
+                    int left = P.max_iter - 1 - it;
+                    bool conv_ul = false;
+                    auto probe = [&]() -> int {
+                        countdown -= 1;
+                        const int fire = countdown == 0;
+                        countdown = fire ? P.check_termination : countdown;
+                        auto lost = [&](const int s, const double vp) {
+                            return (int)(fabs(X[s] - VN[s]) >= P.tol_pri) | (int)(fabs(vp - VN[s]) * rho >= P.tol_dua);
+                        };
+                        const bool maybe = ((int)!(rho > 0.0) | (int)!(lost(UPS0, vp0) | lost(UPS1, vp1))) != 0;
+                        unsigned long long fold = __ballot(maybe);
+                        fold &= fold >> 1; fold &= fold >> 2; fold &= fold >> 4; fold &= fold >> 8;
+                        const bool any_row = (fold & 0x0001000100010001ull) != 0ull;
+                        const bool last_test = left < P.check_termination;
+                        return -fire & ((int)any_row | (int)last_test);
+                    };
+                    auto full_test = [&]() {
+                        double pmax = 0.0, dmax = 0.0;
+#pragma unroll
+                        for (int s = 0; s < N; ++s) {
+                            pmax = resid_max<false>(pmax, X[s] - VN[s]);
+                            dmax = resid_max<false>(dmax, *vp_cell(vcur ^ VSWAP, s) - VN[s]);
+                        }
+                        rp = pmax;
+                        rd = dmax * rho;
+                        const bool ok = (rp < P.tol_pri) && (rd < P.tol_dua);
+                        const unsigned long long bal = __ballot(ok);
+                        conv_ul = ((bal >> (grp * RL)) & RMASK) == RMASK;
+                    };
+                    (void)probe; (void)full_test;
+                    int need = 0;
+                    int again = 0;
+                    bool conv = false;
+                    do {
+                        if constexpr (UL) asm volatile(".p2align 3");
+                        double lvr[LSP ? SPR : 1], lgr[LSP ? SPR : 1], tvr[LTP ? SPR : 1], tgr[LTP ? SPR : 1];
+                        if constexpr (LPL) {
+#pragma unroll
+                            for (int d = 1; d <= SPR && d <= N; ++d) {
+                                if constexpr (LSP) { lvr[(N - d) % SPR] = sLV[cl + (N - d) * CSL]; lgr[(N - d) % SPR] = sLG[cl + (N - d) * CSL]; }
+                                if constexpr (LTP) { tvr[(N - d) % SPR] = sTV[cl + (N - d) * CSL]; tgr[(N - d) % SPR] = sTG[cl + (N - d) * CSL]; }
+                            }
+                        }
+                        auto lin_w = [&](const int s_) { if constexpr (LSP) return lvr[s_ % SPR] - lgr[s_ % SPR]; else return VL[LSR ? s_ : 0] - GL[LSR ? s_ : 0]; };
+                        auto tlin_w = [&](const int s_) { if constexpr (LTP) return tvr[s_ % SPR] - tgr[s_ % SPR]; else return VT[LTR ? s_ : 0] - GT[LTR ? s_ : 0]; };
+                        double qhi;
+                        {
+                            double t = fma(-rho, VN[N - 1] - G[N - 1], QX[N - 1]);
+                            if constexpr (SOC) t = fma(-rho, wr[(N - 1) % SPR], t);
+                            if constexpr (LS) t = fma(-rho, lin_w(N - 1), t);
+                            if constexpr (LT) t = fma(-rho, tlin_w(N - 1), t);
+                            qhi = t;
+                            if constexpr (DBG) {
+                                double ql = fma(-rho, VN[N - 1] - G[N - 1], qx_last_plain);
+                                if constexpr (SOC) ql = fma(-rho, wr[(N - 1) % SPR], ql);
+                                if constexpr (LS) ql = fma(-rho, lin_w(N - 1), ql);
+                                if constexpr (LT) ql = fma(-rho, tlin_w(N - 1), ql);
+                                Qd[N - 1] = is_state ? ql : t;
+                                Pd[N - 1] = t;
+                            }
+                        }
+                        double pcur = qhi;
+                        if constexpr (HALF) {
+                            double tmpv = VN[N - 2] - G[N - 2];
+#pragma unroll
+                            for (int i = N - 2; i >= 0; --i) {
+                                double qlo, res, dnp, tmpn;
+                                constexpr int dummy = 0;
+                                const int in = i > 0 ? i - 1 : dummy;
+                                fused_backward_step_half<NX, NU>(qlo, res, dnp, tmpn, tmpv, VN[in], G[in], QX[i], rho, smask, cb, nim, cf, pcur, qhi, mb, mb + NX);
+                                if (i + 1 <= N - 2) Dn[i + 1] = dnp;
+                                tmpv = tmpn;
+                                pcur = res;
+                                qhi = qlo;
+                            }
+                            Dn[0] = fma(pcur, nim, cf);
+                        }
+#pragma unroll
+                        for (int i = N - 2; i >= 0 && !HALF; --i) {
+                            if constexpr (SOC) {
+                                if (i >= SPD) wr[(i - SPD) % SPR] = sC[cw + (i - SPD) * SLOT_D];
+                            }
+                            if constexpr (LSP) { if (i >= SPD) { lvr[(i - SPD) % SPR] = sLV[cl + (i - SPD) * CSL]; lgr[(i - SPD) % SPR] = sLG[cl + (i - SPD) * CSL]; } }
+                            if constexpr (LTP) { if (i >= SPD) { tvr[(i - SPD) % SPR] = sTV[cl + (i - SPD) * CSL]; tgr[(i - SPD) % SPR] = sTG[cl + (i - SPD) * CSL]; } }
+                            if constexpr (SOC || LPL) __builtin_amdgcn_sched_barrier(0);
+                            if constexpr (FUSED) {
+                                double qlo, res;
+                                if constexpr (SOC) fused_backward_step_soc<NX, NU>(qlo, res, VN[i], G[i], QX[i], wr[i % SPR], rho, smask, cb, pcur, qhi, mb, mb + NX);
+                                else fused_backward_step<NX, NU>(qlo, res, VN[i], G[i], QX[i], rho, smask, cb, pcur, qhi, mb, mb + NX);
+                                pcur = res;
+                                Dn[i] = fma(res, nim, cf);
+                                if constexpr (DBG) { Qd[i] = qlo; Pd[i] = res; Dd[i + 1] = res; }
+                                qhi = qlo;
+                                continue;
+                            }
+                            double qlo = fma(-rho, VN[i] - G[i], QX[i]);
+                            if constexpr (SOC) qlo = fma(-rho, wr[i % SPR], qlo);
+                            if constexpr (LS) qlo = fma(-rho, lin_w(i), qlo);
+                            if constexpr (LT) qlo = fma(-rho, tlin_w(i), qlo);
+                            const double res = ring_sum2<MODE, NX, NU>(fma(qlo, smask, cb), pcur, mb, qhi, mb + NX);
                             pcur = res;
                             Dn[i] = fma(res, nim, cf);
                             if constexpr (DBG) { Qd[i] = qlo; Pd[i] = res; Dd[i + 1] = res; }
                             qhi = qlo;
-                            continue;
-                        }
-                        double qlo = fma(-rho, VN[i] - G[i], QX[i]);
-                        if constexpr (SOC) qlo = fma(-rho, wr[i % SPR], qlo);
-                        if constexpr (LS) qlo = fma(-rho, lin_w(i), qlo);
-                        if constexpr (LT) qlo = fma(-rho, tlin_w(i), qlo);
-                        const double res = ring_sum2<MODE, NX, NU>(fma(qlo, smask, cb), pcur, mb, qhi, mb + NX);
-                        pcur = res;
-                        Dn[i] = fma(res, nim, cf);
-                        if constexpr (DBG) { Qd[i] = qlo; Pd[i] = res; Dd[i + 1] = res; }
-                        qhi = qlo;
-                    }
-                    constexpr bool LAZY_RES = N <= 12;
-                    constexpr bool TIGHT = FUSED && !HALF && LAZY_RES && !SOC && NX % 4 == 0;
-                    double pmax = 0.0, dmax = 0.0;
-                    auto slot_update = [&](const int s, const double lo, const double hi, const double gcv, const double glv, const double gtv) {
-                        const double xi = X[s];
-                        const double t = xi + G[s];
-                        const double vn = TIGHT ? vclamp64(lo, hi, t) : vmin64(hi, vmax64(lo, t));
-                        if constexpr (!LAZY_RES) {
-                            pmax = resid_max<true>(pmax, xi - vn);
-                            dmax = resid_max<true>(dmax, VP[s] - vn);
-                        }
-                        G[s] = t - vn;
-                        VN[s] = vn;
+                        }
+                        double pmax = 0.0, dmax = 0.0;
+                        if constexpr (UL) {
+                            vp0 = __hip_atomic_load(vp_cell(vcur, UPS0), __ATOMIC_RELAXED, __HIP_MEMORY_SCOPE_SINGLETHREAD);
+                            vp1 = __hip_atomic_load(vp_cell(vcur, UPS1), __ATOMIC_RELAXED, __HIP_MEMORY_SCOPE_SINGLETHREAD);
+                        }
+                        auto slot_update = [&](const int s, const double lo, const double hi, const double gcv, const double glv, const double gtv) {
+                            const double xi = X[s];
+                            const double t = xi + G[s];
+                            const double vn = TIGHT ? vclamp64(lo, hi, t) : vmin64(hi, vmax64(lo, t));
+                            if constexpr (!LAZY_RES) {
+                                pmax = resid_max<true>(pmax, xi - vn);
+                                dmax = resid_max<true>(dmax, VP[s] - vn);
+                            }
+                            G[s] = t - vn;
+                            VN[s] = vn;
+                            if constexpr (SOC) {
+                                sC[cw + s * SLOT_D] = fma(xi, socmask, gcv);
+                            }
+                            if constexpr (LSP) sLV[cl + s * CSL] = (lin_lane && (is_state || s >= 1)) ? (xi + glv) : 0.0;
+                            if constexpr (LTP) sTV[cl + s * CSL] = (tlin_lane && (is_state || s >= 1)) ? (xi + gtv) : 0.0;
+                            if constexpr (LSR || LTR) {
+                                auto halfspaces = [&](double z, const double* tabk, const int nk) {
+                                    for (int k = 0; k < nk; ++k) {
+                                        const double a = tabk[k * 16 + j];
+                                        const double bk = tabk[KMAX * 16 + k * 16 + j];
+                                        const double nn = tabk[2 * KMAX * 16 + k * 16 + j];
+                                        const double prod = a * z;
+                                        double cs = 0.0, ci = 0.0;
+                                        ring1<0, NX>(cs, prod, ones);
+                                        ring1<NX, NU>(ci, prod, ones);
+                                        const double cv = is_state ? cs : ci;
+                                        if (cv > bk) {
+#pragma clang fp contract(off)
+                                            const double pr = ((cv - bk) / nn) * a;
+                                            z = z - pr;
+                                        }
+                                    }
+                                    return z;
+                                };
+                                if constexpr (LSR) {
+                                    const bool on = lin_lane && (is_state || s >= 1);
+                                    double vl = on ? (xi + GL[s]) : 0.0;
+                                    vl = halfspaces(vl, rLin, P.n_lin);
+                                    GL[s] = on ? ((GL[s] + xi) - vl) : 0.0;
+                                    VL[s] = on ? vl : 0.0;
+                                }
+                                if constexpr (LTR) {
+                                    const bool on = tlin_lane && (is_state || s >= 1);
+                                    double vt = on ? (xi + GT[s]) : 0.0;
+                                    vt = halfspaces(vt, rTLin + s * 3 * KMAX * 16, P.n_tlin);
+                                    GT[s] = on ? ((GT[s] + xi) - vt) : 0.0;
+                                    VT[s] = on ? vt : 0.0;
+                                }
+                            }
+                        };
+                        double lo_c = UB ? rlo_u0 : sLo[sbox + j], hi_c = UB ? rhi_u0 : sHi[sbox + j];
+                        double gr[SOC ? SPR : 1];
                         if constexpr (SOC) {
-                            sC[cw + s * SLOT_D] = fma(xi, socmask, gcv);
-                        }
-                        if constexpr (LSP) sLV[cl + s * CSL] = (lin_lane && (is_state || s >= 1)) ? (xi + glv) : 0.0;
-                        if constexpr (LTP) sTV[cl + s * CSL] = (tlin_lane && (is_state || s >= 1)) ? (xi + gtv) : 0.0;
-                        if constexpr (LSR || LTR) {
-                            auto halfspaces = [&](double z, const double* tabk, const int nk) {
-                                for (int k = 0; k < nk; ++k) {
-                                    const double a = tabk[k * 16 + j];
-                                    const double bk = tabk[KMAX * 16 + k * 16 + j];
-                                    const double nn = tabk[2 * KMAX * 16 + k * 16 + j];
-                                    const double prod = a * z;
-                                    double cs = 0.0, ci = 0.0;
-                                    ring1<0, NX>(cs, prod, ones);
-                                    ring1<NX, NU>(ci, prod, ones);
-                                    const double cv = is_state ? cs : ci;
-                                    if (cv > bk) {
-#pragma clang fp contract(off)
-                                        const double pr = ((cv - bk) / nn) * a;
-                                        z = z - pr;
+#pragma unroll
+                            for (int d = 0; d < SPD && d < N; ++d) gr[d % SPR] = sC[cw + d * SLOT_D + PL_GC];
+                        } else gr[0] = 0.0;
+                        double glr[LSP ? SPR : 1], gtr[LTP ? SPR : 1];
+                        glr[0] = 0.0; gtr[0] = 0.0;
+                        if constexpr (LPL) {
+#pragma unroll
+                            for (int d = 0; d < SPD && d < N; ++d) {
+                                if constexpr (LSP) glr[d % SPR] = sLG[cl + d * CSL];
+                                if constexpr (LTP) gtr[d % SPR] = sTG[cl + d * CSL];
+                            }
+                        }
+                        double tt_d = 0.0, vn_d = 0.0;
+#pragma unroll
+                        for (int i = 0; i < N - 1; ++i) {
+                            const double lo_n = UB ? rlo_u : sLo[sbox + (i + 1) * 16 + j], hi_n = UB ? rhi_u : sHi[sbox + (i + 1) * 16 + j];
+                            if constexpr (SOC) { if (i + SPD < N) gr[(i + SPD) % SPR] = sC[cw + (i + SPD) * SLOT_D + PL_GC]; }
+                            if constexpr (LSP) { if (i + SPD < N) glr[(i + SPD) % SPR] = sLG[cl + (i + SPD) * CSL]; }
+                            if constexpr (LTP) { if (i + SPD < N) gtr[(i + SPD) % SPR] = sTG[cl + (i + SPD) * CSL]; }
+                            __builtin_amdgcn_sched_barrier(0);
+                            if constexpr (FUSED) {
+                                double tt, vn, xn, t = Dn[i];
+                                const double xi = X[i];
+                                if constexpr (HALF) {
+                                    double gnew;
+                                    fused_forward_step_half<NX, NU>(tt, vn, t, xn, gnew, xi, G[i], lo_c, hi_c, mf1, mf2);
+                                    X[i + 1] = xn;
+                                    if constexpr (!LAZY_RES) {
+                                        pmax = resid_max<true>(pmax, xi - vn);
+                                        dmax = resid_max<true>(dmax, VP[i] - vn);
                                     }
+                                    G[i] = gnew;
+                                    VN[i] = vn;
+                                    lo_c = lo_n; hi_c = hi_n;
+                                    continue;
                                 }
-                                return z;
-                            };
-                            if constexpr (LSR) {
-                                const bool on = lin_lane && (is_state || s >= 1);
-                                double vl = on ? (xi + GL[s]) : 0.0;
-                                vl = halfspaces(vl, rLin, P.n_lin);
-                                GL[s] = on ? ((GL[s] + xi) - vl) : 0.0;
-                                VL[s] = on ? vl : 0.0;
-                            }
-                            if constexpr (LTR) {
-                                const bool on = tlin_lane && (is_state || s >= 1);
-                                double vt = on ? (xi + GT[s]) : 0.0;
-                                vt = halfspaces(vt, rTLin + s * 3 * KMAX * 16, P.n_tlin);
-                                GT[s] = on ? ((GT[s] + xi) - vt) : 0.0;
-                                VT[s] = on ? vt : 0.0;
-                            }
-                        }
-                    };
-                    double lo_c = UB ? rlo_u0 : sLo[sbox + j], hi_c = UB ? rhi_u0 : sHi[sbox + j];
-                    double gr[SOC ? SPR : 1];
-                    if constexpr (SOC) {
-#pragma unroll
-                        for (int d = 0; d < SPD && d < N; ++d) gr[d % SPR] = sC[cw + d * SLOT_D + PL_GC];
-                    } else gr[0] = 0.0;
-                    double glr[LSP ? SPR : 1], gtr[LTP ? SPR : 1];
-                    glr[0] = 0.0; gtr[0] = 0.0;
-                    if constexpr (LPL) {
-#pragma unroll
-                        for (int d = 0; d < SPD && d < N; ++d) {
-                            if constexpr (LSP) glr[d % SPR] = sLG[cl + d * CSL];
-                            if constexpr (LTP) gtr[d % SPR] = sTG[cl + d * CSL];
-                        }
-                    }
-                    double tt_d = 0.0, vn_d = 0.0;
-#pragma unroll
-                    for (int i = 0; i < N - 1; ++i) {
-                        const double lo_n = UB ? rlo_u : sLo[sbox + (i + 1) * 16 + j], hi_n = UB ? rhi_u : sHi[sbox + (i + 1) * 16 + j];
-                        if constexpr (SOC) { if (i + SPD < N) gr[(i + SPD) % SPR] = sC[cw + (i + SPD) * SLOT_D + PL_GC]; }
-                        if constexpr (LSP) { if (i + SPD < N) glr[(i + SPD) % SPR] = sLG[cl + (i + SPD) * CSL]; }
-                        if constexpr (LTP) { if (i + SPD < N) gtr[(i + SPD) % SPR] = sTG[cl + (i + SPD) * CSL]; }
-                        __builtin_amdgcn_sched_barrier(0);
-                        if constexpr (FUSED) {
-                            double tt, vn, xn, t = Dn[i];
-                            const double xi = X[i];
-                            if constexpr (HALF) {
-                                double gnew;
-                                fused_forward_step_half<NX, NU>(tt, vn, t, xn, gnew, xi, G[i], lo_c, hi_c, mf1, mf2);
+                                fused_forward_step<NX, NU, TIGHT>(tt, vn, t, xn, xi, G[i], lo_c, hi_c, mf1, mf2);
                                 X[i + 1] = xn;
                                 if constexpr (!LAZY_RES) {
                                     pmax = resid_max<true>(pmax, xi - vn);
                                     dmax = resid_max<true>(dmax, VP[i] - vn);
                                 }
-                                G[i] = gnew;
+                                if constexpr (TIGHT) {
+                                    __builtin_amdgcn_sched_barrier(0);
+                                    if (i > 0) G[i - 1] = pinned_sub64(tt_d, vn_d);
+                                    tt_d = tt; vn_d = vn;
+                                } else G[i] = tt - vn;
                                 VN[i] = vn;
+                                if constexpr (SOC) sC[cw + i * SLOT_D] = fma(xi, socmask, gr[i % SPR]);
                                 lo_c = lo_n; hi_c = hi_n;
                                 continue;
                             }
-                            fused_forward_step<NX, NU, TIGHT>(tt, vn, t, xn, xi, G[i], lo_c, hi_c, mf1, mf2);
-                            X[i + 1] = xn;
-                            if constexpr (!LAZY_RES) {
-                                pmax = resid_max<true>(pmax, xi - vn);
-                                dmax = resid_max<true>(dmax, VP[i] - vn);
-                            }
-                            if constexpr (TIGHT) {
-                                __builtin_amdgcn_sched_barrier(0);
-                                if (i > 0) G[i - 1] = pinned_sub64(tt_d, vn_d);
-                                tt_d = tt; vn_d = vn;
-                            } else G[i] = tt - vn;
-                            VN[i] = vn;
-                            if constexpr (SOC) sC[cw + i * SLOT_D] = fma(xi, socmask, gr[i % SPR]);
+                            const double t = ring_sum<MODE, 0, NX>(Dn[i], X[i], mf1);
+                            X[i + 1] = ring_short<MODE, NX, NU>(t, t, mf2);
+                            slot_update(i, lo_c, hi_c, gr[SOC ? i % SPR : 0], glr[LSP ? i % SPR : 0], gtr[LTP ? i % SPR : 0]);
                             lo_c = lo_n; hi_c = hi_n;
-                            continue;
-                        }
-                        const double t = ring_sum<MODE, 0, NX>(Dn[i], X[i], mf1);
-                        X[i + 1] = ring_short<MODE, NX, NU>(t, t, mf2);
-                        slot_update(i, lo_c, hi_c, gr[SOC ? i % SPR : 0], glr[LSP ? i % SPR : 0], gtr[LTP ? i % SPR : 0]);
-                        lo_c = lo_n; hi_c = hi_n;
-                    }
-                    if constexpr (TIGHT && N >= 2) G[N - 2] = tt_d - vn_d;
-                    (void)tt_d; (void)vn_d;
-                    slot_update(N - 1, lo_c, hi_c, gr[SOC ? (N - 1) % SPR : 0], glr[LSP ? (N - 1) % SPR : 0], gtr[LTP ? (N - 1) % SPR : 0]);
-                    if constexpr (LPL) {
-                        __builtin_amdgcn_fence(__ATOMIC_RELEASE, "wavefront");
-                        __builtin_amdgcn_wave_barrier();
-                        if constexpr (LSP) {
-                            if (lin_x_on) project_halfspace_columns<NX, KMAX, 16, 16>(j, grp, N, CSL, 0, 0, sLV, sLG, rLin, 0, P.n_lin);
-                            if (lin_u_on) project_halfspace_columns<NU, KMAX, 16, 16>(j, grp, N, CSL, NX, 1, sLV, sLG, rLin, 0, P.n_lin);
-                        }
-                        if constexpr (LTP) {
-                            if (tlin_x_on) project_halfspace_columns<NX, KMAX, 16, 16>(j, grp, N, CSL, 0, 0, sTV, sTG, rTLin, 3 * KMAX * 16, P.n_tlin);
-                            if (tlin_u_on) project_halfspace_columns<NU, KMAX, 16, 16>(j, grp, N, CSL, NX, 1, sTV, sTG, rTLin, 3 * KMAX * 16, P.n_tlin);
-                        }
-                        __builtin_amdgcn_fence(__ATOMIC_RELEASE, "wavefront");
-                        __builtin_amdgcn_wave_barrier();
-                    }
-                    bool conv = false;
-                    auto termination = [&]() {
-                        if (countdown > 0 && --countdown == 0) {
-                            countdown = P.check_termination;
-                            checked = 1;
-                            constexpr int PS0 = N >= 2 ? 1 : 0, PS1 = N - 1;
-                            auto lost = [&](const int s) {
-                                return (int)(fabs(X[s] - VN[s]) >= P.tol_pri) | (int)(fabs(VP[s] - VN[s]) * rho >= P.tol_dua);
-                            };
-                            const bool maybe = ((int)!(rho > 0.0) | (int)!(lost(PS0) | lost(PS1))) != 0;
-                            unsigned long long fold = __ballot(maybe);
-                            fold &= fold >> 1; fold &= fold >> 2; fold &= fold >> 4;
-                            if constexpr (!HALF) fold &= fold >> 8;
-                            const bool any_row = (fold & (HALF ? 0x0101010101010101ull : 0x0001000100010001ull)) != 0ull;
-                            const bool last_test = (P.max_iter - 1 - it) < P.check_termination;
-                            if (last_test || any_row) {
-                                if constexpr (LAZY_RES) {
-#pragma unroll
-                                    for (int s = 0; s < N; ++s) {
-                                        pmax = resid_max<false>(pmax, X[s] - VN[s]);
-                                        dmax = resid_max<false>(dmax, VP[s] - VN[s]);
-                                    }
-                                }
-                                rp = pmax;
-                                rd = dmax * rho;
-                                const bool ok = (rp < P.tol_pri) && (rd < P.tol_dua);
-                                const unsigned long long bal = __ballot(ok);
-                                conv = ((bal >> (grp * RL)) & RMASK) == RMASK;
-                            }
-                        }
-                    };
-                    if constexpr (SOC) {
-                        __builtin_amdgcn_fence(__ATOMIC_RELEASE, "wavefront");
-                        __builtin_amdgcn_wave_barrier();
-                        double n0 = sC[item_at[0]], n1 = sC[item_at[0] + 1], n2 = sC[item_at[0] + 2];
-#pragma unroll
-                        for (int d = 1; d <= SPR && d <= N; ++d) wr[(N - d) % SPR] = sC[cw + (N - d) * SLOT_D];
-                        termination();
-                        bool any_exact = false;
-#pragma unroll
-                        for (int p = 0; p < SOC_PASSES; ++p) {
-                            if (p > 0 && p >= soc_passes) break;
-                            const int at = item_at[p];
-                            if (p > 0) { n0 = sC[at]; n1 = sC[at + 1]; n2 = sC[at + 2]; }
-                            const double s0 = n0, s1 = n1, s2 = n2;
-                            if (soc_all_inside(s0, s1, s2, item_mu[p])) {
-                                sC[at + PL_VC] = s0; sC[at + PL_VC + 1] = s1; sC[at + PL_VC + 2] = s2;
-                                if (!gcz[p]) {
-                                    sC[at + PL_GC] = 0.0; sC[at + PL_GC + 1] = 0.0; sC[at + PL_GC + 2] = 0.0;
-                                    gcz[p] = true;
-                                }
-                            } else {
-                                double r0, r1, r2;
-                                soc_project3(s0, s1, s2, item_mu[p], item_rmu[p], mu_pow2, r0, r1, r2);
-                                const double g0 = s0 - r0, g1 = s1 - r1, g2 = s2 - r2;
-                                sC[at + PL_VC] = r0; sC[at + PL_VC + 1] = r1; sC[at + PL_VC + 2] = r2;
-                                sC[at + PL_GC] = g0; sC[at + PL_GC + 1] = g1; sC[at + PL_GC + 2] = g2;
-                                sC[at] = r0 - g0; sC[at + 1] = r1 - g1; sC[at + 2] = r2 - g2;
-                                gcz[p] = false;
-                                any_exact = true;
-                            }
-                        }
-                        if (it == iter0 && !proj_lane) {
-#pragma unroll
-                            for (int s = 0; s < N; ++s) sC[cw + s * SLOT_D + PL_GC] = 0.0;
-                        }
-                        __builtin_amdgcn_fence(__ATOMIC_RELEASE, "wavefront");
-                        __builtin_amdgcn_wave_barrier();
-                        if (any_exact) {
-#pragma unroll
-                            for (int d = 1; d <= SPR && d <= N; ++d) wr[(N - d) % SPR] = sC[cw + (N - d) * SLOT_D];
-                        }
-                    }
-                    iter += 1;
-                    if constexpr (ADAPT) {
-                        if (it > 0 && it % 5 == 0) {
-                            double at[NX];
-#pragma unroll
-                            for (int k = 0; k < NX; ++k) at[k] = HA ? atab_i[ATAB_AT + k * 16 + j] : sTab[j * AKC + k];
-                            double pri_res = 0.0, ax_max = 0.0, z_max = 0.0, dual_res = 0.0, px_max = 0.0, aty_max = 0.0, q_max = 0.0;
-                            double pxq_max = 0.0;
-#pragma unroll
-                            for (int i = 0; i < N - 1; ++i) {
-                                const double axs = ring_sum<MODE, 0, NX>(0.0, X[i], mf1);
-                                const double dyn = ring_short<MODE, NX, NU>(axs, is_input ? X[i + 1] : 0.0, mf2) - X[i + 1];
-                                const double a = is_state ? dyn : X[i + 1];
-                                const double zz = VN[i + 1];
-                                const bool on = is_state || is_input;
-                                pri_res = fmax(pri_res, on ? fabs(a - zz) : 0.0);
-                                ax_max = fmax(ax_max, on ? fabs(a) : 0.0);
-                                z_max = fmax(z_max, on ? fabs(zz) : 0.0);
-                                const double init = is_state ? (i >= 1 ? -G[i] : 0.0) : G[i + 1];
-                                const double aty = ring_sum<MODE, 0, NX>(init, G[i + 1], at);
-                                const double xs = is_state ? X[i] : X[i + 1];
-                                const double px = qr * xs;
-                                dual_res = fmax(dual_res, on ? fabs((px + px) + aty) : 0.0);
-                                pxq_max = fmax(pxq_max, on ? fabs(px) : 0.0);
-                                aty_max = fmax(aty_max, on ? fabs(aty) : 0.0);
-                            }
-                            {
-                                double prow[NX];
-#pragma unroll
-                                for (int k = 0; k < NX; ++k) prow[k] = sP[grp * NX * NX + (is_state ? j : 0) + NX * k];
-                                const double pxl = ring_sum<MODE, 0, NX>(0.0, X[N - 1], prow);
-                                const double ql = qr * X[N - 1];
-                                const double atyl = -G[N - 1];
-                                dual_res = fmax(dual_res, is_state ? fabs((pxl + ql) + atyl) : 0.0);
-                                px_max = fmax(pxq_max, is_state ? fabs(pxl) : 0.0);
-                                aty_max = fmax(aty_max, is_state ? fabs(atyl) : 0.0);
-                                q_max = fmax(pxq_max, is_state ? fabs(ql) : 0.0);
-                            }
-                            pri_res = grp_max16(pri_res); ax_max = grp_max16(ax_max); z_max = grp_max16(z_max);
-                            dual_res = grp_max16(dual_res); px_max = grp_max16(px_max); aty_max = grp_max16(aty_max); q_max = grp_max16(q_max);
-                            const double pri_norm = fmax(ax_max, z_max);
-                            const double dual_norm = fmax(fmax(px_max, aty_max), q_max);
-                            const double eps = 1e-10;
-                            const double normalized_pri = pri_res / (pri_norm + eps);
-                            const double normalized_dual = dual_res / (dual_norm + eps);
-                            const double ratio = normalized_pri / (normalized_dual + eps);
-                            double new_rho = rho * sqrt(ratio);
-                            if (P.aclip) new_rho = fmin(fmax(new_rho, P.arho_min), P.arho_max);
-                            const double delta = new_rho - rho;
-                            if (is_state) {
-#pragma unroll
-                                for (int k = 0; k < NU; ++k) mb[NX + k] = -taylor_step(-mb[NX + k], delta, (HA ? atab_i[ATAB_DK + k * 16 + j] : sTab[(16 + j) * AKC + k]));
-#pragma unroll
-                                for (int k = 0; k < NX; ++k) {
-                                    const int e = grp * NX * NX + k + NX * j;
-                                    sP[e] = taylor_step(sP[e], delta, (HA ? atab_i[ATAB_DP + k * 16 + j] : sTab[(32 + j) * AKC + k]));
-                                }
-                            } else if (is_input) {
-#pragma unroll
-                                for (int k = 0; k < NX; ++k) mf1[k] = -taylor_step(-mf1[k], delta, (HA ? atab_i[ATAB_DK + k * 16 + j] : sTab[(16 + j) * AKC + k]));
-                            }
-                            if (P.aC1 || P.aC2) {
-                                if (j == 0) sDl[grp * ADAPT_LOG + ndl] = delta;
-                                if (++ndl == ADAPT_LOG) { flush_c(ndl); ndl = 0; }
-                            }
-                            rho = new_rho;
+                        }
+                        if constexpr (TIGHT && N >= 2) G[N - 2] = tt_d - vn_d;
+                        (void)tt_d; (void)vn_d;
+                        slot_update(N - 1, lo_c, hi_c, gr[SOC ? (N - 1) % SPR : 0], glr[LSP ? (N - 1) % SPR : 0], gtr[LTP ? (N - 1) % SPR : 0]);
+                        if constexpr (LPL) {
                             __builtin_amdgcn_fence(__ATOMIC_RELEASE, "wavefront");
                             __builtin_amdgcn_wave_barrier();
-                            QX[N - 1] = qx_last_plain;
-                            terminal_term();
-                        }
+                            if constexpr (LSP) {
+                                if (lin_x_on) project_halfspace_columns<NX, KMAX, 16, 16>(j, grp, N, CSL, 0, 0, sLV, sLG, rLin, 0, P.n_lin);
+                                if (lin_u_on) project_halfspace_columns<NU, KMAX, 16, 16>(j, grp, N, CSL, NX, 1, sLV, sLG, rLin, 0, P.n_lin);
+                            }
+                            if constexpr (LTP) {
+                                if (tlin_x_on) project_halfspace_columns<NX, KMAX, 16, 16>(j, grp, N, CSL, 0, 0, sTV, sTG, rTLin, 3 * KMAX * 16, P.n_tlin);
+                                if (tlin_u_on) project_halfspace_columns<NU, KMAX, 16, 16>(j, grp, N, CSL, NX, 1, sTV, sTG, rTLin, 3 * KMAX * 16, P.n_tlin);
+                            }
+                            __builtin_amdgcn_fence(__ATOMIC_RELEASE, "wavefront");
+                            __builtin_amdgcn_wave_barrier();
+                        }
+                        auto termination = [&]() {
+                            if (countdown > 0 && --countdown == 0) {
+                                countdown = P.check_termination;
+                                checked = 1;
+                                constexpr int PS0 = N >= 2 ? 1 : 0, PS1 = N - 1;
+                                auto lost = [&](const int s) {
+                                    return (int)(fabs(X[s] - VN[s]) >= P.tol_pri) | (int)(fabs(VP[s] - VN[s]) * rho >= P.tol_dua);
+                                };
+                                const bool maybe = ((int)!(rho > 0.0) | (int)!(lost(PS0) | lost(PS1))) != 0;
+                                unsigned long long fold = __ballot(maybe);
+                                fold &= fold >> 1; fold &= fold >> 2; fold &= fold >> 4;
+                                if constexpr (!HALF) fold &= fold >> 8;
+                                const bool any_row = (fold & (HALF ? 0x0101010101010101ull : 0x0001000100010001ull)) != 0ull;
+                                const bool last_test = (P.max_iter - 1 - it) < P.check_termination;
+                                if (last_test || any_row) {
+                                    if constexpr (LAZY_RES) {
+#pragma unroll
+                                        for (int s = 0; s < N; ++s) {
+                                            pmax = resid_max<false>(pmax, X[s] - VN[s]);
+                                            dmax = resid_max<false>(dmax, VP[s] - VN[s]);
+                                        }
+                                    }
+                                    rp = pmax;
+                                    rd = dmax * rho;
+                                    const bool ok = (rp < P.tol_pri) && (rd < P.tol_dua);
+                                    const unsigned long long bal = __ballot(ok);
+                                    conv = ((bal >> (grp * RL)) & RMASK) == RMASK;
+                                }
+                            }
+                        };
+                        if constexpr (SOC) {
+                            __builtin_amdgcn_fence(__ATOMIC_RELEASE, "wavefront");
+                            __builtin_amdgcn_wave_barrier();
+                            double n0 = sC[item_at[0]], n1 = sC[item_at[0] + 1], n2 = sC[item_at[0] + 2];
+#pragma unroll
+                            for (int d = 1; d <= SPR && d <= N; ++d) wr[(N - d) % SPR] = sC[cw + (N - d) * SLOT_D];
+                            termination();
+                            bool any_exact = false;
+#pragma unroll
+                            for (int p = 0; p < SOC_PASSES; ++p) {
+                                if (p > 0 && p >= soc_passes) break;
+                                const int at = item_at[p];
+                                if (p > 0) { n0 = sC[at]; n1 = sC[at + 1]; n2 = sC[at + 2]; }
+                                const double s0 = n0, s1 = n1, s2 = n2;
+                                if (soc_all_inside(s0, s1, s2, item_mu[p])) {
+                                    sC[at + PL_VC] = s0; sC[at + PL_VC + 1] = s1; sC[at + PL_VC + 2] = s2;
+                                    if (!gcz[p]) {
+                                        sC[at + PL_GC] = 0.0; sC[at + PL_GC + 1] = 0.0; sC[at + PL_GC + 2] = 0.0;
+                                        gcz[p] = true;
+                                    }
+                                } else {
+                                    double r0, r1, r2;
+                                    soc_project3(s0, s1, s2, item_mu[p], item_rmu[p], mu_pow2, r0, r1, r2);
+                                    const double g0 = s0 - r0, g1 = s1 - r1, g2 = s2 - r2;
+                                    sC[at + PL_VC] = r0; sC[at + PL_VC + 1] = r1; sC[at + PL_VC + 2] = r2;
+                                    sC[at + PL_GC] = g0; sC[at + PL_GC + 1] = g1; sC[at + PL_GC + 2] = g2;
+                                    sC[at] = r0 - g0; sC[at + 1] = r1 - g1; sC[at + 2] = r2 - g2;
+                                    gcz[p] = false;
+                                    any_exact = true;
+                                }
+                            }
+                            if (it == iter0 && !proj_lane) {
+#pragma unroll
+                                for (int s = 0; s < N; ++s) sC[cw + s * SLOT_D + PL_GC] = 0.0;
+                            }
+                            __builtin_amdgcn_fence(__ATOMIC_RELEASE, "wavefront");
+                            __builtin_amdgcn_wave_barrier();
+                            if (any_exact) {
+#pragma unroll
+                                for (int d = 1; d <= SPR && d <= N; ++d) wr[(N - d) % SPR] = sC[cw + (N - d) * SLOT_D];
+                            }
+                        }
+                        if constexpr (!UL) iter += 1;
+                        if constexpr (ADAPT) {
+                            if (it > 0 && it % 5 == 0) {
+                                double at[NX];
+#pragma unroll
+                                for (int k = 0; k < NX; ++k) at[k] = HA ? atab_i[ATAB_AT + k * 16 + j] : sTab[j * AKC + k];
+                                double pri_res = 0.0, ax_max = 0.0, z_max = 0.0, dual_res = 0.0, px_max = 0.0, aty_max = 0.0, q_max = 0.0;
+                                double pxq_max = 0.0;
+#pragma unroll
+                                for (int i = 0; i < N - 1; ++i) {
+                                    const double axs = ring_sum<MODE, 0, NX>(0.0, X[i], mf1);
+                                    const double dyn = ring_short<MODE, NX, NU>(axs, is_input ? X[i + 1] : 0.0, mf2) - X[i + 1];
+                                    const double a = is_state ? dyn : X[i + 1];
+                                    const double zz = VN[i + 1];
+                                    const bool on = is_state || is_input;
+                                    pri_res = fmax(pri_res, on ? fabs(a - zz) : 0.0);
+                                    ax_max = fmax(ax_max, on ? fabs(a) : 0.0);
+                                    z_max = fmax(z_max, on ? fabs(zz) : 0.0);
+                                    const double init = is_state ? (i >= 1 ? -G[i] : 0.0) : G[i + 1];
+                                    const double aty = ring_sum<MODE, 0, NX>(init, G[i + 1], at);
+                                    const double xs = is_state ? X[i] : X[i + 1];
+                                    const double px = qr * xs;
+                                    dual_res = fmax(dual_res, on ? fabs((px + px) + aty) : 0.0);
+                                    pxq_max = fmax(pxq_max, on ? fabs(px) : 0.0);
+                                    aty_max = fmax(aty_max, on ? fabs(aty) : 0.0);
+                                }
+                                {
+                                    double prow[NX];
+#pragma unroll
+                                    for (int k = 0; k < NX; ++k) prow[k] = sP[grp * NX * NX + (is_state ? j : 0) + NX * k];
+                                    const double pxl = ring_sum<MODE, 0, NX>(0.0, X[N - 1], prow);
+                                    const double ql = qr * X[N - 1];
+                                    const double atyl = -G[N - 1];
+                                    dual_res = fmax(dual_res, is_state ? fabs((pxl + ql) + atyl) : 0.0);
+                                    px_max = fmax(pxq_max, is_state ? fabs(pxl) : 0.0);
+                                    aty_max = fmax(aty_max, is_state ? fabs(atyl) : 0.0);
+                                    q_max = fmax(pxq_max, is_state ? fabs(ql) : 0.0);
+                                }
+                                pri_res = grp_max16(pri_res); ax_max = grp_max16(ax_max); z_max = grp_max16(z_max);
+                                dual_res = grp_max16(dual_res); px_max = grp_max16(px_max); aty_max = grp_max16(aty_max); q_max = grp_max16(q_max);
+                                const double pri_norm = fmax(ax_max, z_max);
+                                const double dual_norm = fmax(fmax(px_max, aty_max), q_max);
+                                const double eps = 1e-10;
+                                const double normalized_pri = pri_res / (pri_norm + eps);
+                                const double normalized_dual = dual_res / (dual_norm + eps);
+                                const double ratio = normalized_pri / (normalized_dual + eps);
+                                double new_rho = rho * sqrt(ratio);
+                                if (P.aclip) new_rho = fmin(fmax(new_rho, P.arho_min), P.arho_max);
+                                const double delta = new_rho - rho;
+                                if (is_state) {
+#pragma unroll
+                                    for (int k = 0; k < NU; ++k) mb[NX + k] = -taylor_step(-mb[NX + k], delta, (HA ? atab_i[ATAB_DK + k * 16 + j] : sTab[(16 + j) * AKC + k]));
+#pragma unroll
+                                    for (int k = 0; k < NX; ++k) {
+                                        const int e = grp * NX * NX + k + NX * j;
+                                        sP[e] = taylor_step(sP[e], delta, (HA ? atab_i[ATAB_DP + k * 16 + j] : sTab[(32 + j) * AKC + k]));
+                                    }
+                                } else if (is_input) {
+#pragma unroll
+                                    for (int k = 0; k < NX; ++k) mf1[k] = -taylor_step(-mf1[k], delta, (HA ? atab_i[ATAB_DK + k * 16 + j] : sTab[(16 + j) * AKC + k]));
+                                }
+                                if (P.aC1 || P.aC2) {
+                                    if (j == 0) sDl[grp * ADAPT_LOG + ndl] = delta;
+                                    if (++ndl == ADAPT_LOG) { flush_c(ndl); ndl = 0; }
+                                }
+                                rho = new_rho;
+                                __builtin_amdgcn_fence(__ATOMIC_RELEASE, "wavefront");
+                                __builtin_amdgcn_wave_barrier();
+                                QX[N - 1] = qx_last_plain;
+                                terminal_term();
+                            }
+                        }
+                        if constexpr (UL) {
+                            need = probe();
+                            const int vnext = vcur ^ VSWAP;
+#pragma unroll
+                            for (int s = 0; s < N; ++s)
+                                __hip_atomic_store(vp_cell(vnext, s), VN[s], __ATOMIC_RELAXED, __HIP_MEMORY_SCOPE_SINGLETHREAD);
+                            vcur = vnext;
+                            again = (need == 0 && left > 0) ? 1 : 0;
+                            left -= again;
+                        }
+                        if constexpr (!SOC && !UL) termination();
+                    } while (UL && again != 0);
+                    if constexpr (UL) {
+                        it = P.max_iter - 1 - left;
+                        iter = it + 1;
+                        if (need) full_test();
+                        if (conv_ul) { vcur ^= VSWAP; solved = 1; break; }
+                        continue;
                     }
-                    if constexpr (!SOC) termination();
                     if (conv) { solved = 1; break; }
 #pragma unroll
                     for (int s = 0; s < N; ++s) VP[s] = VN[s];
                     vp_touched = true;
+                }
+                if constexpr (UL) {
+                    vp_touched = vp_touched || (iter - iter0 - solved) > 0;
+                    if (P.check_termination > 0 && iter - iter0 >= P.check_termination) checked = 1;
                 }
                 acc_iter += (unsigned)(iter - iter0);
                 acc_solved += (unsigned)solved;
@@ -1371,7 +1444,8 @@
                         const double xs = is_input ? (s + 1 < N ? X[s + 1 < N ? s + 1 : s] : 0.0) : X[s];
                         const double vs = is_input ? (s + 1 < N ? VN[s + 1 < N ? s + 1 : s] : 0.0) : VN[s];
                         const double gs = is_input ? (s + 1 < N ? G[s + 1 < N ? s + 1 : s] : 0.0) : G[s];
-                        const double ps = is_input ? (s + 1 < N ? VP[s + 1 < N ? s + 1 : s] : 0.0) : VP[s];
+                        const double ps = UL ? (is_input ? (s + 1 < N ? *vp_cell(vcur, s + 1 < N ? s + 1 : s) : 0.0) : *vp_cell(vcur, s))
+                                             : (is_input ? (s + 1 < N ? VP[s + 1 < N ? s + 1 : s] : 0.0) : VP[s]);
                         if (in_row) {
                             if (P.store_mask & 1) {
                                 if (acc_iter > 0) { if constexpr (PF) P.prim[off] = xs; else store_primal(P.prim + off, xs); }
@@ -1395,7 +1469,7 @@
                     }
                     if (P.store_mask & 2) P.slack[off] = VN[s];
                     if (P.store_mask & 4) P.dual[off] = G[s];
-                    if ((P.store_mask & 8) && vp_touched) P.slack_prev[off] = VP[s];
+                    if ((P.store_mask & 8) && vp_touched) P.slack_prev[off] = UL ? *vp_cell(vcur, s) : VP[s];
                     if constexpr (SOC) {
                         if (soc_lane && (P.store_mask & 16)) {
                             P.cslack[off] = sC[cw + s * SLOT_D + ((proj_lane || iter <= iter_first) ? PL_VC : 0)];
```

Result: slower. 2.674 billion QP solves/s (-6.7%).
